# achraf-15/HiDeNN-FEM

Hardware: AMD Instinct MI355X
Metric: element-evals/sec (fwd+bwd energy) + achieved HBM GB/s, 2D quad mesh (higher is better)
Workload: dtype f64; 1 GPU; Example 4 (T1M x 1): 2D plate linear elasticity, 1000000 TRI3 (structured quads split in 2), 501501 nodes, gauss_order=4, r-adaptivity on, Neumann edges 500, fwd+bwd (loss + dX + dU); elements=1000000, nodes=501501, elements_per_gpu=1000000, tiles=1024, tile_elems=1200, element_order=paired slots, threads_per_tile=256, lds_bytes=38784, launch=hipgraph (1 x 1000 steps + 1 x 290), exchange=none, full=False

## Files before the change

hidenn_fem_amd/_lib.py:

```python
from __future__ import annotations

import ctypes as C
import os

import torch

_HERE = os.path.dirname(os.path.abspath(__file__))
LIB_PATH = os.path.join(_HERE, "csrc", "libhidenn_hip_lab.so" if os.environ.get("HFEM_LAB") == "1" else "libhidenn_hip.so")

_vp = C.c_void_p
_i32, _i64, _f64 = C.c_int32, C.c_int64, C.c_double


class PlanStats(C.Structure):
    _fields_ = [
        ("n_elems", _i64), ("n_nodes", _i64), ("n_edges", _i64),
        ("n_tiles", _i32), ("tile_elems", _i32),
        ("tile_elem_total", _i64), ("tile_node_total", _i64),
        ("max_tile_nodes", _i32), ("max_tile_owned", _i32),
        ("max_tile_elems", _i32), ("max_tile_edges", _i32),
        ("device_bytes", _i64), ("lds_bytes", _i32),
        ("shards", _i32), ("threads_per_tile", _i32), ("paired", _i32), ("slot_rows", _i32),
        ("store_policy", _i32), ("nodes_per_elem", _i32), ("row_line_factor", _f64),
    ]

    def as_dict(self):
        return {k: getattr(self, k) for k, _ in self._fields_}


class AdamTensor(C.Structure):
    _fields_ = [("p", _vp), ("g", _vp), ("m", _vp), ("v", _vp), ("n", _i64), ("lr", _f64), ("beta1", _f64),
                ("beta2", _f64), ("eps", _f64), ("dtype", _i32), ("block_begin", _i32)]


ADAM_TICKET_INTS = 1056


PROTOTYPES = {
    "hfem_version": (C.c_int, []),
    "hfem_last_error": (C.c_char_p, []),
    "hfem_device_count": (C.c_int, []),
    "hfem_tri3_energy_atomic": (C.c_int, [C.c_int, _vp, _vp, _vp, _i64, _i64, _i64, _vp, _f64, _vp, _vp, _vp, _vp, _vp]),
    "hfem_edge2_energy_atomic": (C.c_int, [C.c_int, _vp, _vp, _vp, _i64, _vp, _vp, _vp, _vp, _vp, _vp]),
    "hfem_plan_create": (C.c_int, [C.c_int, _vp, _i64, _i64, _vp, _vp, _vp, _vp, _i64, _i32, C.POINTER(_vp)]),
    "hfem_plan_create_ex": (C.c_int, [C.c_int, _vp, _i64, _i64, _i32, _vp, _vp, _vp, _vp, _i64, _i32, C.POINTER(_vp)]),
    "hfem_plan_destroy": (C.c_int, [_vp]),
    "hfem_plan_get_stats": (C.c_int, [_vp, C.POINTER(PlanStats)]),
    "hfem_plan_export": (_i64, [_vp, C.c_int, _vp, _i64]),
    "hfem_plan_serialize": (_i64, [_vp, _vp, _i64]),
    "hfem_plan_deserialize": (C.c_int, [C.c_int, _vp, _i64, C.POINTER(_vp)]),
    "hfem_tri3_energy_plan": (C.c_int, [_vp, _vp, _vp, _vp, _vp, _vp, _f64, _vp, _vp, _vp, _i32, _i32, _vp, _vp, _vp, _i32, _vp]),
    "hfem_tri3_energy_plan_f32": (C.c_int, [_vp, _vp, _vp, _vp, _vp, _vp, _f64, _vp, _vp, _vp, _i32, _i32, _vp, _vp, _vp, _i32, _vp]),
    "hfem_set_option": (C.c_int, [C.c_char_p, C.c_int]),
    "hfem_get_option": (C.c_int, [C.c_char_p]),
    "hfem_tri3_eval_fwd": (C.c_int, [C.c_int, _vp, _vp, _vp, _vp, _vp, _i64, _vp, _vp, _vp, _vp]),
    "hfem_tri3_eval_bwd": (C.c_int, [C.c_int, _vp, _vp, _vp, _vp, _vp, _i64, _vp, _vp, _vp, _vp, _vp, _vp]),
    "hfem_tri3_eval_fwd_conv": (C.c_int, [C.c_int, _vp, _vp, _vp, _vp, _vp, _i64, _vp, _vp, _vp, _i32, _vp]),
    "hfem_tri3_eval_bwd_conv": (C.c_int, [C.c_int, _vp, _vp, _vp, _vp, _vp, _i64, _vp, _vp, _vp, _vp, _vp, _i32, _vp]),
    "hfem_edge2_eval_fwd": (C.c_int, [C.c_int, _vp, _vp, _vp, _vp, _vp, _i64, _vp, _vp, _vp]),
    "hfem_edge2_eval_bwd": (C.c_int, [C.c_int, _vp, _vp, _vp, _vp, _vp, _i64, _vp, _vp, _vp, _vp, _vp]),
    "hfem_quad4_energy_atomic": (C.c_int, [C.c_int, _vp, _vp, _vp, _i64, _i64, _i64, _vp, _vp, _vp, _vp, _vp]),
    "hfem_adam_step_dev": (C.c_int, [C.c_int, _vp, _vp, _vp, _vp, _i64, _i32, C.c_double, C.c_double, C.c_double,
                                     C.c_double, _vp, _vp]),
    "hfem_counter_add": (C.c_int, [C.c_int, _vp, _i64, _vp]),
    "hfem_adam_multi_dev": (C.c_int, [C.c_int, _vp, _i32, _i32, _i64, _vp, _i64, _vp, _vp]),
    "hfem_lbfgs_create": (C.c_int, [C.c_int, _i64, _i32, _i32, C.POINTER(_vp)]),
    "hfem_lbfgs_destroy": (C.c_int, [_vp]),
    "hfem_lbfgs_check": (C.c_int, [_vp, _vp, _vp, _i32, C.c_double, C.c_double, _vp, _vp]),
    "hfem_lbfgs_direction": (C.c_int, [_vp, _vp, C.c_double, C.c_double, _vp]),
    "hfem_lbfgs_apply": (C.c_int, [_vp, _vp, _i64, _i64, _vp]),
    "hfem_lbfgs_direction_ptr": (_vp, [_vp]),
    "hfem_lbfgs_shard_payload_doubles": (_i64, [_vp]),
    "hfem_lbfgs_shard_gather": (C.c_int, [_vp, _vp, _vp, _i64, _vp, _vp, _i64, _vp, _vp]),
    "hfem_lbfgs_shard_local": (C.c_int, [_vp, _vp, _vp, _vp, _vp]),
    "hfem_lbfgs_shard_finish": (C.c_int, [_vp, _vp, _vp, _i32, _i32, _i32, _f64, _f64, _f64, _vp, _vp]),
    "hfem_lbfgs_shard_apply": (C.c_int, [_vp, _vp, _vp, _i64, _vp, _vp, _i64, _vp]),
    "hfem_lbfgs_shard_status": (C.c_int, [_vp, _vp, _vp]),
    "hfem_tri3_von_mises": (C.c_int, [C.c_int, _vp, _vp, _vp, _i64, C.c_double, C.c_double, _vp, _vp, _vp]),
    "hfem_line2_slopes": (C.c_int, [C.c_int, _vp, _vp, _i64, _i32, _vp, _vp]),
    "hfem_quad4_von_mises": (C.c_int, [C.c_int, _vp, _vp, _vp, _i64, C.c_double, C.c_double, _vp, _vp, _vp]),
    "hfem_tri3_stress_recover": (C.c_int, [C.c_int, _vp, _vp, _vp, _i64, _i64, _vp, _vp, _vp, _i32, _vp, _vp, _vp]),
    "hfem_quad4_stress_recover": (C.c_int, [C.c_int, _vp, _vp, _vp, _i64, _i64, _vp, _vp, _vp, _i32, _vp, _vp, _vp]),
    "hfem_tri3_zz_error": (C.c_int, [C.c_int, _vp, _vp, _vp, _i64, _vp, _vp, _i32, _vp, _vp, _vp, _vp, _vp]),
    "hfem_quad4_zz_error": (C.c_int, [C.c_int, _vp, _vp, _vp, _i64, _vp, _vp, _i32, _vp, _vp, _vp, _vp, _vp]),
    "hfem_tri3_hyper_energy_plan": (C.c_int, [_vp, _i32, _vp, _vp, _vp, _vp, _vp, _f64, _vp, _vp, _vp, _vp, _vp, _vp, _vp, _vp,
                                              _i32, _vp]),
    "hfem_quad4_hyper_energy_plan": (C.c_int, [_vp, _i32, _vp, _vp, _vp, _vp, _vp, _vp, _vp, _vp, _vp, _vp, _vp, _vp, _vp, _i32,
                                               _vp]),
    "hfem_tri3_energy_adam_step": (C.c_int, [_vp, _vp, _vp, _vp, _vp, _vp, _f64, _vp, _vp, _vp, _vp, _vp, _vp, _vp, _vp,
                                             _f64, _f64, _f64, _f64, _f64, _vp, _vp, _i32, _vp]),
    "hfem_tri3_energy_adam_step_ex": (C.c_int, [_vp, _i32, _vp, _vp, _vp, _vp, _vp, _f64, _vp, _vp, _vp, _vp, _vp, _vp, _vp, _vp,
                                                _vp, _f64, _f64, _f64, _f64, _f64, _vp, _i32, _i32, _vp, _i32, _vp]),
    "hfem_adam_prep": (C.c_int, [C.c_int, _vp, _f64, _f64, _vp, _vp]),
    "hfem_plan_loss_sum": (C.c_int, [_vp, _i32, _i32, _vp, _vp]),
    "hfem_iface_pack": (C.c_int, [C.c_int, _vp, _vp, _vp, _i32, _i32, _vp, _vp]),
    "hfem_iface_unpack": (C.c_int, [C.c_int, _vp, _vp, _vp, _i32, _i32, _vp, _vp, _i32, _i64, _i64, _vp, _vp]),
    "hfem_mg_load": (C.c_int, [C.c_char_p]),
    "hfem_mg_unique_id": (C.c_int, [_vp]),
    "hfem_mg_comm_create": (C.c_int, [C.c_int, C.c_int, C.c_int, _vp, C.POINTER(_vp)]),
    "hfem_mg_comm_destroy": (C.c_int, [_vp]),
    "hfem_mg_allreduce_sum": (C.c_int, [_vp, _vp, _vp, _i64, _vp]),
    "hfem_mg_allgather": (C.c_int, [_vp, _vp, _vp, _i64, _vp]),
    "hfem_adam_step_rows_dev": (C.c_int, [C.c_int, _vp, _vp, _vp, _vp, _vp, _i64, _f64, _f64, _f64, _f64, _vp, _vp]),
    "hfem_plan_set_span_stamps": (C.c_int, [_vp, _vp, _i64]),
    "hfem_peer_create": (C.c_int, [C.c_int, _i32, _i32, _i64, C.POINTER(_vp)]),
    "hfem_peer_ipc_handle": (C.c_int, [_vp, _vp]),
# ... 150 lines not shown
```

hidenn_fem_amd/csrc/build.py:

```python
from __future__ import annotations

import os
import subprocess
import sys
from concurrent.futures import ThreadPoolExecutor

HERE = os.path.dirname(os.path.abspath(__file__))
ROOT = os.path.dirname(os.path.dirname(HERE))
SOURCES = ["plan.cpp", "mg.cpp", "tri3_energy.hip", "tri3_stream.hip", "tri3_pair.hip", "tri3_pair_f32.hip", "tri3_pair_lab.hip", "tri3_pair_pipe.hip", "tri3_det.hip", "tri3_eval.hip", "line_rect.hip", "quad4.hip", "optim.hip", "exchange.hip", "peer.hip", "post.hip", "recover.hip", "lbfgs.hip", "cg.hip", "tri3_cg.hip", "quad4_cg.hip", "mesh_guard.hip", "amg.cpp", "tri3_amg.hip", "tri3_hyper.hip", "tri3_hyper_cg.hip", "quad4_hyper.hip", "quad4_hyper_cg.hip", "modal.hip"]
HEADERS = ["hfem_common.h", "hfem_amg.h", "hfem_amg_hyper_dev.h", "hfem_cg_dev.h", "hfem_crossing_dev.h", "hfem_device.h", "hfem_hyper_dev.h", "hfem_mesh_dev.h", "hfem_mesh_elem_dev.h", "hfem_plan_dev.h", "hfem_quad4_dev.h", "hfem_quad4_hyper_dev.h", "hfem_recover_hyper_dev.h", "tri3_energy_lab.inc", os.path.join(ROOT, "include", "hidenn_fem.h")]
OUT = os.path.join(HERE, "libhidenn_hip.so")
OUT_LAB = os.path.join(HERE, "libhidenn_hip_lab.so")
ARCH = "gfx950"
CXXFLAGS = ["-O3", "-std=c++17", "-fPIC", f"--offload-arch={ARCH}", "-munsafe-fp-atomics",
            "-ffp-contract=on", "-Wall", "-Wno-unused-function"]


def _stale(target, deps):
    if not os.path.exists(target):
        return True
    t = os.path.getmtime(target)
    return any(os.path.getmtime(d) > t for d in deps)


def build(force: bool = False, keep_temps: bool = False, lab: bool = False, tag: str = "", defines=()) -> str:
    hipcc = os.environ.get("HIPCC", "/opt/rocm/bin/hipcc")
    bdir = os.path.join(HERE, "build", "lab") if lab else os.path.join(HERE, "build")
    out = OUT_LAB if lab else OUT
    flags = CXXFLAGS + (["-DHFEM_LAB"] if lab else [])
    if tag:
        bdir, out = os.path.join(HERE, "build", tag), os.path.join(HERE, f"libhidenn_hip_{tag}.so")
        flags = flags + ["-D" + d for d in defines]
    srcs = [os.path.join(HERE, s) for s in SOURCES]
    hdrs = [h if os.path.isabs(h) else os.path.join(HERE, h) for h in HEADERS]
    objs = [os.path.join(bdir, os.path.splitext(s)[0] + ".o") for s in SOURCES]
    os.makedirs(bdir, exist_ok=True)

    def compile_one(pair):
        src, obj = pair
        res = obj + ".resource.txt"
        if not force and not _stale(obj, [src] + hdrs + [__file__]) and os.path.exists(res):
            return
        cmd = [hipcc] + flags + ["-x", "hip", "-c", src, "-o", obj, "-Rpass-analysis=kernel-resource-usage"]
        if keep_temps:
            cmd += ["-save-temps=obj"]
        r = subprocess.run(cmd, capture_output=True, text=True, cwd=bdir)
        if r.returncode != 0:
            raise RuntimeError(f"hipcc failed for {src}:\n{r.stdout}\n{r.stderr}")
        with open(res, "w") as f:
            f.write(r.stderr)

    with ThreadPoolExecutor(max_workers=4) as ex:
        list(ex.map(compile_one, zip(srcs, objs)))
    if force or _stale(out, objs):
        cmd = [hipcc, "-shared", "-fPIC", f"--offload-arch={ARCH}", "-o", out] + objs
        r = subprocess.run(cmd, capture_output=True, text=True)
        if r.returncode != 0:
            raise RuntimeError(f"link failed:\n{r.stdout}\n{r.stderr}")
    return out


def resource_usage(lab: bool = False):
    import re
    bdir = os.path.join(HERE, "build", "lab") if lab else os.path.join(HERE, "build")
    out = {}
    for s in SOURCES:
        path = os.path.join(bdir, os.path.splitext(s)[0] + ".o.resource.txt")
        if not os.path.exists(path):
            raise RuntimeError(f"{path} missing: run build() first")
        text = open(path).read()
        for blk in text.split("Function Name: ")[1:]:
            name = blk.split()[0]
            get = lambda key: int(re.search(key + r": (\d+)", blk).group(1))
            out[name] = dict(vgprs=get(r" VGPRs"), scratch=get(r"ScratchSize \[bytes/lane\]"), occupancy=get(r"Occupancy \[waves/SIMD\]"),
                             source=s)
    return out


if __name__ == "__main__":
    tag = sys.argv[sys.argv.index("--tag") + 1] if "--tag" in sys.argv else ""
    defs = [sys.argv[i + 1] for i, v in enumerate(sys.argv) if v == "--define"]
    print(build(force="--force" in sys.argv, keep_temps="--keep-temps" in sys.argv, lab="--lab" in sys.argv, tag=tag, defines=defs))
```

hidenn_fem_amd/csrc/hfem_common.h:

```cpp
#pragma once
#include <cstdint>
#include <cstdio>
#include <string>
#include <vector>

#include "../../include/hidenn_fem.h"

namespace hfem {

void set_error(const std::string &msg);
const char *get_error();

#define HFEM_ARG_CHECK(cond, msg)                                            \
    do {                                                                     \
        if (!(cond)) {                                                       \
            ::hfem::set_error(std::string(__func__) + ": " + (msg));         \
            return -1;                                                       \
        }                                                                    \
    } while (0)

constexpr int kLocalBits = 10;
constexpr int kMaxLocal = 1 << kLocalBits;
constexpr uint32_t kLocalMask = kMaxLocal - 1;
constexpr uint32_t kHomeBit = 1u << 30;
constexpr uint32_t kSkipBit = 1u << 31;
constexpr uint32_t kHasBBit = 1u << 10;
constexpr uint32_t kHomeBBit = 1u << 11;
constexpr uint32_t kChainedBit = 1u << 12;
constexpr int32_t kNodeTailPad = 2048;
constexpr int32_t kElemTailPad = 4096;
constexpr int32_t kMaxQuadSlots = 1024;

struct TileDesc {
    int32_t elem_off, n_elem;
    int32_t node_off, n_node;
    int32_t n_owned;
    int32_t edge_off, n_edge;
    int32_t pad;
};
static_assert(sizeof(TileDesc) == 32, "TileDesc must be 8 x int32");

struct HostPlan {
    int64_t ne = 0, nn = 0, ned = 0;
    int32_t tile_elems = 0;
    int32_t npe = 3;
    std::vector<TileDesc> tiles;
    std::vector<uint32_t> elem_pack;
    std::vector<uint32_t> elem_pack_hi;
    std::vector<int32_t> elem_gid;
    std::vector<int32_t> node_src;
    int32_t node_stride = 0, elem_stride = 0;
    int64_t elem_records = 0;
    int32_t col_stride = 0;
    int64_t node_records = 0;
    std::vector<uint32_t> edge_pack;
    std::vector<int32_t> edge_gid;
    int32_t max_nodes = 0, max_owned = 0, max_elems = 0, max_edges = 0;
    std::vector<int32_t> tile_chunks;
    std::vector<int32_t> elem_gid_b;
    bool paired = false;
    int64_t n_pairs = 0, n_chained = 0;
    int32_t max_rows = 0;
    std::vector<int32_t> conn32, x_src_g, u_src_g, edges32;
    int32_t max_chunk_elems = 0;
    int32_t shards = 1;
    std::vector<int32_t> shard_desc;
    int32_t pair_block = 256;
    std::vector<int32_t> owned_gid;
    std::vector<int32_t> owned_gid_by_slot;
};
constexpr int kChunks = 3;

int build_host_plan(const int64_t *conn, int npe, int64_t ne, int64_t nn, const double *coords,
                    const int32_t *x_src, const int32_t *u_src, const int64_t *edges,
                    int64_t ned, int32_t tile_elems, int32_t node_cap, int elem_order, int32_t chunk_cap,
                    HostPlan &out, int32_t pair_block = 256, int32_t shards = 1);

void serialize_host_plan(const HostPlan &h, const void *trailer, size_t trailer_bytes, std::vector<unsigned char> &blob);
int deserialize_host_plan(const void *blob, size_t n, HostPlan &h, void *trailer, size_t trailer_bytes);

void set_plan_curve(int c);
void set_plan_read_pack(int v);
void set_plan_snap(int percent);

}
```

hidenn_fem_amd/csrc/hfem_plan_dev.h:

```cpp
#pragma once
#include <hip/hip_runtime.h>

#include <mutex>
#include <vector>

#include "hfem_device.h"

namespace hfem {

struct PlanDev {
    const TileDesc *tiles;
    const uint32_t *elem_pack;
    const int2 *node_src;
    const uint32_t *edge_pack;
    const int32_t *edge_gid;
    const uint32_t *elem_pack_hi;
    const int4 *tile_chunks;
    int node_stride;
    int elem_stride;
    unsigned long long *span;
};

constexpr int kMaxPeers = 16;
constexpr size_t kPeerFlags = 0, kPeerData = 256;
// ... 201 lines not shown
    const int q = nb >> 3, r = nb & 7, x = b & 7;
    return x * q + min(x, r) + (b >> 3);
}

}

namespace hfem {
constexpr int kPipeMaxTiles = 16;
}

struct hfem_plan {
    hfem::HostPlan host;
    int device = -1;
    hfem::TileDesc *d_tiles = nullptr;
    uint32_t *d_elem_pack = nullptr;
    uint32_t *d_elem_pack_hi = nullptr;
    int2 *d_node_src = nullptr;
    uint32_t *d_edge_pack = nullptr;
    int32_t *d_edge_gid = nullptr;
    int4 *d_tile_chunks = nullptr;
    struct Det {
        int32_t *conn = nullptr, *x_src = nullptr, *u_src = nullptr, *edges = nullptr;
        int32_t *adj_ptr = nullptr, *adj = nullptr, *eadj_ptr = nullptr, *eadj = nullptr;
        double *partials = nullptr;
        int n_blocks = 0;
        bool ready = false;
    } det;
    double *d_partials = nullptr;
    std::mutex mu;
    int bank = 0;
    int prev_begin = 0, prev_n = 0;
    void *prev_stream = nullptr;
    struct Tune { int tiled_block = 512, store_policy = 16, tiled_fast = 1, fast_const_caps = 1, pair_tiles_per_wg = 1, pair_pipe_wps = 4; } tune;
    unsigned long long *d_stamps = nullptr;
    unsigned long long *span_buf = nullptr;
    int64_t span_slots = 0, span_next = 0;
    int64_t device_bytes = 0;
    double row_line_factor = 1.0;
    const hfem::PeerGetDev *peer_get = nullptr;
    const hfem::PeerPutDev *peer_put = nullptr;
    double *put_bc[2] = {nullptr, nullptr};
    const int32_t *put_pos[2] = {nullptr, nullptr};
    int peer_wait_begin = 0, peer_wait_end = 0;
    int32_t lds_bytes = 0;
    int32_t lds_bytes_pipe = 0;
};

namespace hfem {
inline PlanDev plan_dev(const hfem_plan *p) {
    return PlanDev{p->d_tiles, p->d_elem_pack, p->d_node_src, p->d_edge_pack, p->d_edge_gid, p->d_elem_pack_hi, p->d_tile_chunks, p->host.node_stride, p->host.elem_stride, nullptr};
}
inline Tri3Consts make_consts(const double mat[4], double W, const double Bk[6]) {
    Tri3Consts k;
    k.c11 = mat[0]; k.c12 = mat[1]; k.c22 = mat[2]; k.c33 = mat[3];
    k.W = W;
    for (int i = 0; i < 6; ++i) k.Bk[i] = Bk ? Bk[i] : 0.0;
    return k;
}
int launch_tri3_stream(const hfem_plan *plan, int n_grid, int tile_begin, const double *x_free, const double *x_fixed,
                       const double *u_free, const double *u_fixed, const Tri3Consts &kc, const double *T_edge,
                       double4 tc, double *partials, double *gx_free, double *gu_free, int skip_edges, int store_policy,
                       const LagSum &lag, hipStream_t s, int ablate = 0);
struct TileLaunch {
    PlanDev pd;
    int grid = 0, tile_begin = 0;
    const void *x_free = nullptr, *x_fixed = nullptr, *u_free = nullptr, *u_fixed = nullptr;
    Tri3Consts k;
    const double4 *T_edge = nullptr;
    double4 tc;
    double *partials = nullptr;
    void *gx = nullptr, *gu = nullptr;
    int max_nodes = 0, max_owned = 0, skip_edges = 0;
    int chain = -1;
    int lab_bits = 0;
    int col_stride = 256;
    unsigned long long *span = nullptr;
    unsigned long long *stamps = nullptr;
    size_t lds = 0;
    hipStream_t s = nullptr;
    int stagger = 0, stagger_cfg = 0x108;
};
int launch_tri3_pair(const hfem_plan *plan, TileLaunch A, int mode, bool hasb, bool phys, const LagSum &lag,
                     const AdamFuse &af);
int launch_tri3_pair_f32(const hfem_plan *plan, TileLaunch A, bool hasb, const LagSum &lag, const AdamFuse *adam = nullptr);
#ifdef HFEM_LAB
int launch_tri3_pair_lab(const hfem_plan *plan, TileLaunch A, int mode, bool hasb, bool phys, const LagSum &lag,
                         const AdamFuse &af);
#endif
int launch_tri3_pair_pipe(const hfem_plan *plan, TileLaunch A, int n_tiles, int tpw, const LagSum &lag);
int launch_tri3_det(hfem_plan *plan, const double *x_free, const double *x_fixed, const double *u_free,
                    const double *u_fixed, const Tri3Consts &kc, const double *T_edge, double4 tc, double *loss_out,
                    double *gx_free, double *gu_free, int skip_edges, bool phys, hipStream_t s);
void free_tri3_det(hfem_plan *plan);
int det_prepare(hfem_plan *plan, hipStream_t s);
int launch_iface_pack_sum(int dtype, const void *x_free, const void *u_free, const int32_t *rows, int n_x, int n_u, double *out,
                          int64_t loss_slot, const double *partials, int n_partials, int64_t *counter, double beta1,
                          double beta2, double *bc_next, hipStream_t s);
int launch_iface_put(const hfem_peer *peer, int dtype, const void *x_free, const void *u_free, const int32_t *rows, int n_x,
                     int n_u, int64_t loss_slot, const double *partials, int n_partials, int64_t *counter, double beta1,
                     double beta2, double *bc_next, hipStream_t s);
}
struct hfem_peer {
    int device = -1;
    int64_t stride = 0;
    size_t bytes = 0;
    char *local = nullptr;
    char *ctl = nullptr;
    hfem::PeerGetDev *get_dev = nullptr;
    hfem::PeerPutDev *put_dev = nullptr;
    const int32_t *put_pos[2] = {nullptr, nullptr};
    std::vector<void *> opened;
    bool connected = false;
    hfem::PeerView view{};
};
namespace hfem {
extern int g_quad4_stagger, g_quad4_stagger_shift, g_quad4_stagger_groups;
extern int g_quad4_ablate, g_quad4_pipe, g_quad4_const_caps, g_quad4_bits;

}
```

hidenn_fem_amd/csrc/plan.cpp:

```cpp
#include <algorithm>
#include <array>
#include <atomic>
#include <unordered_map>
#include <cstring>
#include <limits>
#include <numeric>

#include "hfem_common.h"

namespace hfem {

static thread_local std::string g_err;
void set_error(const std::string &msg) { g_err = msg; }
const char *get_error() { return g_err.c_str(); }

namespace {

inline uint32_t spread16(uint32_t v) {
    v &= 0xFFFFu;
    v = (v | (v << 8)) & 0x00FF00FFu;
    v = (v | (v << 4)) & 0x0F0F0F0Fu;
    v = (v | (v << 2)) & 0x33333333u;
    v = (v | (v << 1)) & 0x55555555u;
    return v;
// ... 344 lines not shown
            }
        telems.swap(out);
        return;
    }
    std::vector<std::vector<int32_t>> batch(nb);
    std::vector<std::vector<uint64_t>> used(nb, std::vector<uint64_t>(kMaxLocal / 64, 0));
    std::vector<int32_t> leftover;
    int start = 0;
    for (int i = 0; i < n; ++i) {
        const int32_t e = telems[i];
        int32_t l[3];
        for (int k = 0; k < 3; ++k) l[k] = lid[conn[3 * (int64_t)e + k]];
        int placed = -1;
        for (int t = 0; t < nb; ++t) {
            const int b = (start + t) % nb;
            const int cap = (b == nb - 1) ? n - 64 * (nb - 1) : 64;
            if ((int)batch[b].size() >= cap) continue;
            bool clash = false;
            for (int k = 0; k < 3; ++k)
                if (l[k] < n_owned && (used[b][l[k] >> 6] >> (l[k] & 63)) & 1) clash = true;
            if (clash) continue;
            placed = b;
            break;
        }
        if (placed < 0) { leftover.push_back(e); continue; }
        batch[placed].push_back(e);
        for (int k = 0; k < 3; ++k)
            if (l[k] < n_owned) used[placed][l[k] >> 6] |= 1ull << (l[k] & 63);
        start = (placed + 1) % nb;
    }
    size_t lo = 0;
    for (int b = 0; b < nb; ++b) {
        const int cap = (b == nb - 1) ? n - 64 * (nb - 1) : 64;
        while ((int)batch[b].size() < cap && lo < leftover.size()) batch[b].push_back(leftover[lo++]);
        out.insert(out.end(), batch[b].begin(), batch[b].end());
    }
    telems.swap(out);
}

void cut_tiles(const int64_t *conn, int npe, int64_t ne, int64_t nn, const std::vector<int32_t> &order, int32_t T,
               int32_t node_cap, std::vector<int64_t> &bounds) {
    bounds.assign(1, 0);
    if (node_cap <= 0) {
        for (int64_t p = T; p < ne; p += T) bounds.push_back(p);
        bounds.push_back(ne);
        return;
    }
    std::vector<int32_t> stamp(nn, -1);
    int32_t tile = 0, distinct = 0;
    int64_t start = 0;
    for (int64_t p = 0; p < ne; ++p) {
        const int64_t e = order[p];
        int fresh = 0;
        for (int k = 0; k < npe; ++k)
            if (stamp[conn[npe * e + k]] != tile) ++fresh;
        if (p > start && (p - start >= T || distinct + fresh > node_cap)) {
            int64_t cut = p;
            if (g_snap > 0 && (int64_t)g_codes.size() == ne) {
                const int64_t lo = std::max(start + 1, p - ((p - start) * g_snap) / 100);
                int best_lvl = -1;
                for (int64_t q = p; q >= lo; --q) {
                    const uint32_t x = g_codes[q - 1] ^ g_codes[q];
                    const int lvl = x ? (31 - __builtin_clz(x)) / 2 : -1;
                    if (lvl > best_lvl) { best_lvl = lvl; cut = q; }
                }
            }
            bounds.push_back(cut);
            ++tile;
            start = cut;
            distinct = 0;
            if (cut != p) { p = cut - 1; continue; }
        }
        for (int k = 0; k < npe; ++k) {
            int32_t &st = stamp[conn[npe * e + k]];
            if (st != tile) { st = tile; ++distinct; }
        }
    }
    bounds.push_back(ne);
}

int try_build(const int64_t *conn, int npe, int64_t ne, int64_t nn, const double *xy, const int32_t *x_src,
              const int32_t *u_src, const int64_t *edges, int64_t ned, int32_t T, int32_t node_cap,
              const std::vector<int32_t> &order, int elem_order, int32_t chunk_cap, int32_t pair_block, int32_t shards,
              HostPlan &P) {
    std::vector<int64_t> bounds;
    cut_tiles(conn, npe, ne, nn, order, T, node_cap, bounds);
    const int32_t nt_main = ne > 0 ? (int32_t)bounds.size() - 1 : 0;
    std::vector<int32_t> tile_of(ne);
    for (int32_t t = 0; t < nt_main; ++t)
        for (int64_t p = bounds[t]; p < bounds[t + 1]; ++p) tile_of[p] = t;
    std::vector<int32_t> owner(nn, std::numeric_limits<int32_t>::max());
    for (int64_t p = 0; p < ne; ++p) {
        const int32_t t = tile_of[p];
        const int64_t e = order[p];
        for (int k = 0; k < npe; ++k) {
            int32_t &o = owner[conn[npe * e + k]];
            if (t < o) o = t;
        }
    }
    int64_t n_orphan = 0;
    for (int64_t n = 0; n < nn; ++n)
        if (owner[n] == std::numeric_limits<int32_t>::max())
            owner[n] = nt_main + (int32_t)(n_orphan++ / kOrphanTileNodes);
    const int32_t nt = nt_main + (int32_t)((n_orphan + kOrphanTileNodes - 1) / kOrphanTileNodes);

    if (shards < 1) shards = 1;
    std::vector<int32_t> shard_of(nt, 0);
    std::vector<char> bnd(nt, 0);
    for (int32_t r = 0; r < shards; ++r)
        for (int64_t t = ((int64_t)nt * r) / shards; t < ((int64_t)nt * (r + 1)) / shards; ++t) shard_of[t] = r;

    std::vector<int64_t> adj_ptr(nn + 1, 0);
    for (int64_t e = 0; e < ne; ++e)
        for (int k = 0; k < npe; ++k) adj_ptr[conn[npe * e + k] + 1]++;
    for (int64_t n = 0; n < nn; ++n) adj_ptr[n + 1] += adj_ptr[n];
    std::vector<int32_t> adj(adj_ptr[nn]);
    {
        std::vector<int64_t> fill(adj_ptr.begin(), adj_ptr.end() - 1);
        for (int64_t p = 0; p < ne; ++p) {
            const int32_t e = order[p];
            for (int k = 0; k < npe; ++k) adj[fill[conn[npe * e + k]]++] = e;
        }
    }
    std::vector<int32_t> home(ne);
    for (int64_t p = 0; p < ne; ++p) home[order[p]] = tile_of[p];

    std::vector<int64_t> own_ptr(nt + 1, 0), edg_ptr(nt + 1, 0);
    for (int64_t n = 0; n < nn; ++n) own_ptr[owner[n] + 1]++;
    for (int64_t g = 0; g < ned; ++g) {
        const int32_t ti = owner[edges[2 * g]], tj = owner[edges[2 * g + 1]];
        edg_ptr[ti + 1]++;
        if (tj != ti) edg_ptr[tj + 1]++;
    }
    for (int32_t t = 0; t < nt; ++t) { own_ptr[t + 1] += own_ptr[t]; edg_ptr[t + 1] += edg_ptr[t]; }
    std::vector<int32_t> own(nn), tedge(edg_ptr[nt]);
    {
        std::vector<int64_t> f(own_ptr.begin(), own_ptr.end() - 1);
        for (int64_t n = 0; n < nn; ++n) own[f[owner[n]]++] = (int32_t)n;
        std::vector<int64_t> fe(edg_ptr.begin(), edg_ptr.end() - 1);
        for (int64_t g = 0; g < ned; ++g) {
            const int32_t ti = owner[edges[2 * g]], tj = owner[edges[2 * g + 1]];
            tedge[fe[ti]++] = (int32_t)g;
            if (tj != ti) tedge[fe[tj]++] = (int32_t)g;
        }
    }

    P = HostPlan();
    P.ne = ne; P.nn = nn; P.ned = ned; P.tile_elems = T; P.npe = npe;
    P.tiles.resize(nt);
    P.elem_pack.reserve(ne + ne / 4);
    P.elem_gid.reserve(ne + ne / 4);
    P.node_src.reserve(2 * (nn + nn / 3));

    bool by_row = false;
    if (x_src) {
        int32_t last = -1;
        for (int64_t n = 0; n < nn && !by_row; ++n)
            if (x_src[n] >= 0) { by_row = x_src[n] < last; last = x_src[n]; }
    }
    auto row_key = [&](int32_t n) -> int64_t { return x_src[n] >= 0 ? (int64_t)x_src[n] : ((int64_t)1 << 32) + (int64_t)(~x_src[n]); };
    auto by_row_less = [&](int32_t a, int32_t b) { return row_key(a) < row_key(b); };
    std::vector<int32_t> stamp_e(ne, -1), stamp_n(nn, -1), lid(nn, 0);
    std::vector<int32_t> first_use_stamp(elem_order == 4 ? nn : 0, -1), first_use(elem_order == 4 ? nn : 0, 0);
    std::vector<int32_t> telems, halo, own_order_buf;
    for (int32_t t = 0; t < nt; ++t) {
        TileDesc &d = P.tiles[t];
        d = TileDesc();
// ... 54 lines not shown
                    }
                    const bool along_x = (hi[0] - lo[0]) >= (hi[1] - lo[1]);
                    for (int i = 0; i < n; ++i) key[i] = {along_x ? cx[i] : cy[i], i};
                } else {
                    for (int i = 0; i < n; ++i) key[i] = {(double)i, i};
                }
                std::stable_sort(key.begin(), key.end());
                for (int r = 0; r < n; ++r) strip_of[key[r].second] = (int32_t)(((int64_t)r * kChunks) / std::max(n, 1));
            }
            for (int i = 0; i < n; ++i)
                for (int k = 0; k < npe; ++k) {
                    const int32_t nd = (int32_t)conn[npe * (int64_t)telems[i] + k];
                    if (first_use_stamp[nd] != t) { first_use_stamp[nd] = t; first_use[nd] = strip_of[i]; }
                    else first_use[nd] = std::min(first_use[nd], strip_of[i]);
                }
            auto fu = [&](int32_t nd) { return first_use_stamp[nd] == t ? first_use[nd] : kChunks - 1; };
            auto by_use = [&](int32_t a, int32_t b) { const int32_t fa = fu(a), fb = fu(b); return fa != fb ? fa < fb : a < b; };
            std::sort(own_order.begin(), own_order.end(), by_use);
            std::sort(halo.begin(), halo.end(), by_use);
            nloc = 0;
            for (int32_t nd : own_order) lid[nd] = nloc++;
            int32_t cnt_o[kChunks] = {0}, cnt_h[kChunks] = {0};
            for (int32_t nd : own_order) cnt_o[fu(nd)]++;
            for (int32_t nd : halo) cnt_h[fu(nd)]++;
            for (int32_t nd : halo) lid[nd] = nloc++;
            std::vector<int32_t> packed, part;
            int32_t ends[kChunks];
            for (int c = 0; c < kChunks; ++c) {
                part.clear();
                for (int i = 0; i < n; ++i)
                    if (strip_of[i] == c) part.push_back(telems[i]);
                pack_bank_groups(part, conn, npe, lid, d.n_owned, true, true, packed);
                ends[c] = (int32_t)packed.size();
                const int32_t len = ends[c] - (c ? ends[c - 1] : 0);
                if (chunk_cap > 0 && len > chunk_cap) return 1;
                P.max_chunk_elems = std::max(P.max_chunk_elems, len);
            }
            telems.swap(packed);
            const int32_t po0 = (cnt_o[0] + 63) / 64, po1 = (cnt_o[0] + cnt_o[1] + 63) / 64;
            const int32_t ph0 = (cnt_h[0] + 63) / 64, ph1 = (cnt_h[0] + cnt_h[1] + 63) / 64;
            chunk_rec[0] = ends[0]; chunk_rec[1] = ends[1];
            chunk_rec[2] = po0 | (po1 << 8) | (ph0 << 16) | (ph1 << 24);
        } else {
            for (int32_t n : halo) lid[n] = nloc++;
            if (!(elem_order >= 5 && npe == 3)) order_tile_elements(telems, conn, npe, lid, d.n_owned, elem_order);
        }
        nloc = d.n_owned + (int32_t)halo.size();
        if (elem_order == 4) P.tile_chunks.insert(P.tile_chunks.end(), chunk_rec, chunk_rec + 4);

        d.elem_off = (int32_t)P.elem_pack.size();
        d.node_off = (int32_t)(P.node_src.size() / 2);
        d.n_node = nloc;
        d.edge_off = (int32_t)P.edge_pack.size();
        d.n_edge = (int32_t)(edg_ptr[t + 1] - edg_ptr[t]);
        if (elem_order >= 5 && npe == 3) {
            const int n = (int)telems.size();
            std::unordered_map<uint64_t, int32_t> by_edge0;
            by_edge0.reserve((size_t)n * 2);
            for (int i = 0; i < n; ++i) {
                const int64_t e = telems[i];
                by_edge0[((uint64_t)conn[3 * e] << 32) | (uint32_t)conn[3 * e + 1]] = i;
            }
            std::vector<int32_t> succ(n, -1), pred(n, -1);
            for (int i = 0; i < n; ++i) {
                const int64_t e = telems[i];
                auto it = by_edge0.find(((uint64_t)conn[3 * e] << 32) | (uint32_t)conn[3 * e + 2]);
                if (it != by_edge0.end() && it->second != i && pred[it->second] < 0) { succ[i] = it->second; pred[it->second] = i; }
            }
            std::vector<char> used(n, 0);
            std::vector<std::array<int32_t, 2>> slots;
            slots.reserve(n);
            for (int pass = 0; pass < 2; ++pass)
                for (int i = 0; i < n; ++i) {
                    if (used[i] || (pass == 0 && pred[i] >= 0)) continue;
                    int a = i;
                    while (a >= 0 && !used[a]) {
                        used[a] = 1;
                        const int b = succ[a];
                        if (b >= 0 && !used[b]) { used[b] = 1; slots.push_back({a, b}); a = succ[b]; }
                        else { slots.push_back({a, -1}); a = -1; }
                    }
                }
            std::stable_sort(slots.begin(), slots.end(), [](const std::array<int32_t, 2> &x, const std::array<int32_t, 2> &y) { return (x[1] >= 0) > (y[1] >= 0); });
            std::vector<std::array<int32_t, 4>> items(slots.size());
            for (size_t s_ = 0; s_ < slots.size(); ++s_) {
                const int64_t ea = telems[slots[s_][0]];
                items[s_] = {lid[conn[3 * ea]], lid[conn[3 * ea + 1]], lid[conn[3 * ea + 2]],
                             slots[s_][1] >= 0 ? lid[conn[3 * (int64_t)telems[slots[s_][1]] + 2]] : -1};
            }
            std::vector<int32_t> order_s;
            std::vector<char> chain(slots.size(), 0);
            size_t n_pair = 0;
            while (n_pair < slots.size() && slots[n_pair][1] >= 0) ++n_pair;
            d.pad = pair_block;
            if (elem_order == 6 && pair_block != 256) { set_error("plan: the strip order (lab) needs 256-thread tiles"); return -1; }
            if (elem_order == 6) {
                const int S = (int)slots.size();
                const int H = std::min(kMaxRows, std::max(1, (S + 255) / 256));
                if (S > 256 * kMaxRows) return 1;
                auto gnode = [&](int si, int k) -> int64_t {
                    return k < 3 ? conn[3 * (int64_t)telems[slots[si][0]] + k] : conn[3 * (int64_t)telems[slots[si][1]] + 2];
                };
                std::unordered_map<uint64_t, int32_t> by_nd;
                by_nd.reserve(n_pair * 2);
                for (size_t si = 0; si < n_pair; ++si) by_nd[((uint64_t)gnode((int)si, 0) << 32) | (uint32_t)gnode((int)si, 3)] = (int32_t)si;
                std::vector<int32_t> nxt(n_pair, -1), prv(n_pair, -1);
                for (size_t si = 0; si < n_pair; ++si) {
                    auto it = by_nd.find(((uint64_t)gnode((int)si, 1) << 32) | (uint32_t)gnode((int)si, 2));
                    if (it != by_nd.end() && it->second != (int32_t)si && prv[it->second] < 0) { nxt[si] = it->second; prv[it->second] = (int32_t)si; }
                }
                std::vector<std::vector<int32_t>> strips, columns;
                {
                    const int L = H;
                    strips.clear();
                    std::vector<char> seen(n_pair, 0);
                    for (int pass = 0; pass < 2; ++pass)
                        for (size_t si = 0; si < n_pair; ++si) {
                            if (seen[si] || (pass == 0 && prv[si] >= 0)) continue;
                            int32_t a = (int32_t)si;
                            while (a >= 0 && !seen[a]) {
                                strips.emplace_back();
                                while (a >= 0 && !seen[a] && (int)strips.back().size() < L) { seen[a] = 1; strips.back().push_back(a); a = nxt[a]; }
                            }
                        }
                    std::stable_sort(strips.begin(), strips.end(), [](const std::vector<int32_t> &x, const std::vector<int32_t> &y) { return x.size() > y.size(); });
                    for (size_t si = n_pair; si < slots.size(); ++si) strips.push_back({(int32_t)si});
                    const int ncol = (S + H - 1) / H;
                    columns.assign(ncol, {});
                    std::vector<std::vector<int32_t>> with_room(H + 1);
                    for (int ci = ncol - 1; ci >= 0; --ci) with_room[H].push_back(ci);
                    for (size_t k = 0; k < strips.size(); ++k) {
                        std::vector<int32_t> st = strips[k];
                        while (!st.empty()) {
                            const int len = (int)st.size();
                            int r = len;
                            while (r <= H && with_room[r].empty()) ++r;
                            int take = len;
                            if (r > H) {
                                r = len - 1;
                                while (r > 0 && with_room[r].empty()) --r;
                                take = r;
                            }
                            if (r <= 0) return -1;
                            const int32_t ci = with_room[r].back();
                            with_room[r].pop_back();
                            columns[ci].insert(columns[ci].end(), st.begin(), st.begin() + take);
                            for (int q = 0; q + 1 < take; ++q) chain[st[q]] = 1;
                            if (r - take > 0) with_room[r - take].push_back(ci);
                            st.erase(st.begin(), st.begin() + take);
                        }
                    }
                    while (!columns.empty() && columns.back().empty()) columns.pop_back();
                }
                if (columns.size() > 256) return 1;
                auto shape = [&](const std::vector<int32_t> &c) { uint32_t v = 0; for (int32_t si : c) v = v * 4 + (chain[si] ? 3u : (slots[si][1] >= 0 ? 2u : 1u)); for (size_t q = c.size(); q < (size_t)kMaxRows; ++q) v *= 4; return v; };
                std::stable_sort(columns.begin(), columns.end(), [&](const std::vector<int32_t> &x, const std::vector<int32_t> &y) {
                    const uint32_t sx = shape(x), sy = shape(y);
                    return sx != sy ? sx > sy : gnode(x[0], 0) < gnode(y[0], 0);
                });
                std::vector<std::array<int32_t, 4 * kMaxRows>> citems(columns.size());
                int rows_used = 0;
                for (size_t ci = 0; ci < columns.size(); ++ci) {
                    citems[ci].fill(-1);
                    rows_used = std::max(rows_used, (int)columns[ci].size());
                    for (size_t r = 0; r < columns[ci].size(); ++r) {
                        const int32_t si = columns[ci][r];
                        citems[ci][4 * r + 0] = items[si][0];
                        citems[ci][4 * r + 3] = items[si][3];
                        if (!chain[si]) { citems[ci][4 * r + 1] = items[si][1]; citems[ci][4 * r + 2] = items[si][2]; }
                    }
                }
                std::vector<int32_t> corder;
                pack_column_groups(citems, d.n_owned, corder);
                const int stride = (int)((corder.size() + 15) / 16 * 16);
                d.pad = stride;
                order_s.assign((size_t)rows_used * stride, -1);
                for (size_t t_ = 0; t_ < corder.size(); ++t_)
                    for (size_t r = 0; r < columns[corder[t_]].size(); ++r) order_s[r * stride + t_] = columns[corder[t_]][r];
                while (!order_s.empty() && order_s.back() < 0) order_s.pop_back();
                P.max_rows = std::max(P.max_rows, rows_used);
            } else {
            if (g_halfwave_pack) {
                pack_slot_halfwaves(items, d.n_owned, order_s);
            } else {
                std::vector<std::array<int32_t, 4>> part(items.begin(), items.begin() + n_pair);
                std::vector<int32_t> o;
                pack_slot_groups(part, d.n_owned, o);
                while (!o.empty() && (o.size() & 15)) o.push_back(-1);
                order_s = o;
                part.assign(items.begin() + n_pair, items.end());
                o.clear();
                pack_slot_groups(part, d.n_owned, o);
                for (int32_t v : o) order_s.push_back(v < 0 ? -1 : v + (int32_t)n_pair);
            }
            P.max_rows = std::max(P.max_rows, ((int)order_s.size() + pair_block - 1) / pair_block);
            }
            d.n_elem = (int32_t)order_s.size();
            for (int32_t si : order_s) {
                if (si < 0) {
                    P.elem_pack.push_back(kSkipBit);
                    P.elem_pack_hi.push_back(0u);
                    P.elem_gid.push_back(-1);
                    P.elem_gid_b.push_back(-1);
                    continue;
                }
                const int32_t ea = telems[slots[si][0]], eb = slots[si][1] >= 0 ? telems[slots[si][1]] : -1;
                const std::array<int32_t, 4> &L = items[si];
                P.elem_pack.push_back((uint32_t)L[0] | ((uint32_t)L[1] << kLocalBits) | ((uint32_t)L[2] << (2 * kLocalBits)) |
                                      (home[ea] == t ? kHomeBit : 0u));
                P.elem_pack_hi.push_back(eb >= 0 ? ((uint32_t)L[3] | kHasBBit | (home[eb] == t ? kHomeBBit : 0u) | (chain[si] ? kChainedBit : 0u)) : 0u);
                P.elem_gid.push_back(ea);
                P.elem_gid_b.push_back(eb);
                P.n_pairs += eb >= 0;
                P.n_chained += chain[si];
            }
            P.paired = true;
        } else {
        d.n_elem = (int32_t)telems.size();
        for (int32_t e : telems) {
            if (e < 0) {
                P.elem_pack.push_back(kSkipBit);
                if (npe == 4) P.elem_pack_hi.push_back(0u);
                P.elem_gid.push_back(-1);
                continue;
            }
            const uint32_t l0 = lid[conn[npe * (int64_t)e]], l1 = lid[conn[npe * (int64_t)e + 1]],
                           l2 = lid[conn[npe * (int64_t)e + 2]];
            P.elem_pack.push_back(l0 | (l1 << kLocalBits) | (l2 << (2 * kLocalBits)) |
                                  (home[e] == t ? kHomeBit : 0u));
            if (npe == 4) P.elem_pack_hi.push_back((uint32_t)lid[conn[npe * (int64_t)e + 3]]);
            P.elem_gid.push_back(e);
        }
        }
        auto push_node = [&](int32_t n) {
            P.node_src.push_back(x_src ? x_src[n] : n);
            P.node_src.push_back(u_src ? u_src[n] : n);
        };
        for (int32_t n : own_order) { push_node(n); P.owned_gid_by_slot.push_back(n); }
        for (int32_t n : halo) { push_node(n); P.owned_gid_by_slot.push_back(n); }
        for (int64_t i = edg_ptr[t]; i < edg_ptr[t + 1]; ++i) {
            const int32_t g = tedge[i];
            const int64_t ni = edges[2 * (int64_t)g], nj = edges[2 * (int64_t)g + 1];
            P.edge_pack.push_back((uint32_t)lid[ni] | ((uint32_t)lid[nj] << kLocalBits) |
                                  (owner[ni] == t ? kHomeBit : 0u));
            P.edge_gid.push_back(g);
        }
        P.max_nodes = std::max(P.max_nodes, d.n_node);
        P.max_owned = std::max(P.max_owned, d.n_owned);
        P.max_elems = std::max(P.max_elems, d.n_elem);
        P.max_edges = std::max(P.max_edges, d.n_edge);
    }
    P.shards = shards;
    P.pair_block = pair_block;
    P.shard_desc.clear();
    {
        std::vector<TileDesc> sorted_tiles;
        std::vector<int32_t> sorted_chunks;
        const bool has_chunks = P.tile_chunks.size() == (size_t)4 * nt;
        sorted_tiles.reserve(nt);
        auto take = [&](int32_t t) {
            sorted_tiles.push_back(P.tiles[t]);
            if (has_chunks) sorted_chunks.insert(sorted_chunks.end(), P.tile_chunks.begin() + 4 * (size_t)t, P.tile_chunks.begin() + 4 * (size_t)t + 4);
        };
        for (int32_t r = 0; r < shards; ++r) {
            const int32_t lo = (int32_t)(((int64_t)nt * r) / shards), hi = (int32_t)(((int64_t)nt * (r + 1)) / shards);
            for (int32_t t = lo; t < hi; ++t)
                if (bnd[t]) take(t);
            const int32_t mid = (int32_t)sorted_tiles.size();
            for (int32_t t = lo; t < hi; ++t)
                if (!bnd[t]) take(t);
            P.shard_desc.insert(P.shard_desc.end(), {lo, mid, hi, 0});
        }
        if (shards > 1) {
            P.tiles.swap(sorted_tiles);
            if (has_chunks) P.tile_chunks.swap(sorted_chunks);
        }
    }
    {
        std::vector<int32_t> og;
        og.reserve(nn);
        for (const TileDesc &d : P.tiles)
            for (int32_t l = 0; l < d.n_owned; ++l) og.push_back(P.owned_gid_by_slot[(size_t)d.node_off + l]);
        P.owned_gid.swap(og);
    }
    {
        const int32_t stride = std::max(16, (P.max_nodes + 15) / 16 * 16);
        if ((int64_t)nt * stride + kNodeTailPad > (int64_t)std::numeric_limits<int32_t>::max()) {
            set_error("plan: tile arrays exceed int32 offsets");
            return -1;
        }
        std::vector<int32_t> ns((size_t)2 * ((size_t)nt * stride + kNodeTailPad));
        int32_t lastx = 0, lastu = 0;
        for (int32_t t = 0; t < nt; ++t) {
            TileDesc &d = P.tiles[t];
            const int32_t *srcp = P.node_src.data() + 2 * (size_t)d.node_off;
            int32_t *dst = ns.data() + 2 * (size_t)t * stride;
            std::memcpy(dst, srcp, sizeof(int32_t) * 2 * (size_t)d.n_node);
            if (d.n_node > 0) { lastx = srcp[2 * (d.n_node - 1)]; lastu = srcp[2 * (d.n_node - 1) + 1]; }
            else if (t == 0 && nt > 1 && P.tiles[1].n_node > 0) { lastx = P.node_src[2 * (size_t)P.tiles[1].node_off]; lastu = P.node_src[2 * (size_t)P.tiles[1].node_off + 1]; }
            for (int32_t l = d.n_node; l < stride; ++l) { dst[2 * l] = lastx; dst[2 * l + 1] = lastu; }
            d.node_off = t * stride;
        }
        for (size_t l = (size_t)nt * stride; l < (size_t)nt * stride + kNodeTailPad; ++l) { ns[2 * l] = lastx; ns[2 * l + 1] = lastu; }
        P.node_records = (int64_t)P.node_src.size() / 2;
        P.node_src.swap(ns);
        P.node_stride = stride;
    }
    {
        int32_t cs = 0;
        if (P.paired) {
            for (int32_t t = 0; t < nt; ++t) cs = std::max(cs, P.tiles[t].pad);
            P.max_elems = 0;
            for (int32_t t = 0; t < nt; ++t) {
                const TileDesc &d = P.tiles[t];
                const int32_t ne_new = d.n_elem > 0 ? ((d.n_elem - 1) / d.pad) * cs + (d.n_elem - 1) % d.pad + 1 : 0;
                P.max_elems = std::max(P.max_elems, ne_new);
            }
            P.col_stride = cs;
        }
        const int64_t stride = std::max(16, (P.max_elems + 15) / 16 * 16);
        const size_t total = (size_t)nt * stride + kElemTailPad;
        if (total > (size_t)std::numeric_limits<int32_t>::max()) { set_error("plan: tile arrays exceed int32 offsets"); return -1; }
        const bool hi = !P.elem_pack_hi.empty(), gb = !P.elem_gid_b.empty();
        std::vector<uint32_t> ep(total, kSkipBit), eh(hi ? total : 0, 0u);
        std::vector<int32_t> eg(total, -1), egb(gb ? total : 0, -1);
        int64_t real = 0;
        for (int32_t t = 0; t < nt; ++t) {
            TileDesc &d = P.tiles[t];
            const size_t so = (size_t)d.elem_off, dn = (size_t)t * stride, n = (size_t)d.n_elem;
            int32_t n_new = 0;
            for (size_t i = 0; i < n; ++i) {
                const size_t k = cs > 0 ? (i / d.pad) * cs + i % d.pad : i;
                ep[dn + k] = P.elem_pack[so + i];
                eg[dn + k] = P.elem_gid[so + i];
                if (hi) eh[dn + k] = P.elem_pack_hi[so + i];
                if (gb) egb[dn + k] = P.elem_gid_b[so + i];
                n_new = (int32_t)k + 1;
            }
            real += d.n_elem;
            d.elem_off = (int32_t)dn;
            d.n_elem = n_new;
            if (cs > 0) d.pad = cs;
        }
        P.elem_pack.swap(ep); P.elem_gid.swap(eg); P.elem_pack_hi.swap(eh); P.elem_gid_b.swap(egb);
        P.elem_stride = (int32_t)stride;
        P.elem_records = real;
    }
    if (P.elem_pack.size() > (size_t)std::numeric_limits<int32_t>::max() ||
        P.node_src.size() / 2 > (size_t)std::numeric_limits<int32_t>::max()) {
        set_error("plan: tile arrays exceed int32 offsets");
        return -1;
    }
    return 0;
}

}

void set_plan_curve(int c) { set_locality_curve(c); }
void set_plan_snap(int percent) { set_tile_snap(percent); }
void set_plan_read_pack(int v) { set_halfwave_pack(v); }

int build_host_plan(const int64_t *conn, int npe, int64_t ne, int64_t nn, const double *coords,
                    const int32_t *x_src, const int32_t *u_src, const int64_t *edges,
                    int64_t ned, int32_t tile_elems, int32_t node_cap, int elem_order, int32_t chunk_cap,
                    HostPlan &out, int32_t pair_block, int32_t shards) {
    if (pair_block != 256 && pair_block != 512) { set_error("plan: pair_block must be 256 or 512"); return -1; }
    if (shards < 1 || shards > 4096) { set_error("plan: shards must be in [1, 4096]"); return -1; }
    if (npe != 3 && npe != 4) { set_error("plan: nodes per element must be 3 (TRI3) or 4 (QUAD4)"); return -1; }
    if (ne < 0 || nn < 0 || ned < 0 || nn > std::numeric_limits<int32_t>::max() ||
        ne > std::numeric_limits<int32_t>::max() || ned > std::numeric_limits<int32_t>::max()) {
        set_error("plan: sizes must be in [0, 2^31)");
        return -1;
    }
    if ((ne > 0 && !conn) || (ned > 0 && !edges)) { set_error("plan: null connectivity/edges"); return -1; }
    for (int64_t i = 0; i < npe * ne; ++i)
        if (conn[i] < 0 || conn[i] >= nn) { set_error("plan: connectivity index out of range"); return -1; }
    for (int64_t i = 0; i < 2 * ned; ++i)
        if (edges[i] < 0 || edges[i] >= nn) { set_error("plan: edge index out of range"); return -1; }
    if (tile_elems <= 0) tile_elems = 1024;
    if (tile_elems > 4096) tile_elems = 4096;

    std::vector<int32_t> order;
    morton_order(conn, npe, ne, nn, coords, order);
    for (int32_t T = tile_elems; T >= 16; T = (T * 2) / 3) {
        const int rc = try_build(conn, npe, ne, nn, coords, x_src, u_src, edges, ned, T, node_cap, order, elem_order, chunk_cap,
                                 pair_block, shards, out);
        if (rc == 0 && npe == 4 && out.max_elems > kMaxQuadSlots) continue;
        if (rc == 0 && out.paired && out.max_rows > (pair_block == 512 ? 2 : kMaxRows)) continue;
        if (rc == 0) {
            out.conn32.assign(conn, conn + npe * ne);
            out.edges32.assign(edges, edges + 2 * ned);
            out.x_src_g.resize(nn);
            out.u_src_g.resize(nn);
            for (int64_t n = 0; n < nn; ++n) {
                out.x_src_g[n] = x_src ? x_src[n] : (int32_t)n;
                out.u_src_g[n] = u_src ? u_src[n] : (int32_t)n;
            }
        }
        if (rc <= 0) return rc;
    }
    set_error("plan: could not fit a tile into 1024 local nodes / element slots (node valence too high?)");
    return -1;
}

namespace {
constexpr uint32_t kBlobVersion = 1;
struct BlobScalars {
    int64_t ne, nn, ned, elem_records, node_records, n_pairs, n_chained;
    int32_t tile_elems, npe, node_stride, elem_stride, col_stride, max_nodes, max_owned, max_elems, max_edges, max_rows,
        max_chunk_elems, shards, pair_block, paired;
};
uint64_t fnv1a(const unsigned char *p, size_t n) {
    uint64_t h = 1469598103934665603ull;
    size_t i = 0;
    for (; i + 8 <= n; i += 8) {
        uint64_t w;
        std::memcpy(&w, p + i, 8);
        h = (h ^ w) * 1099511628211ull;
    }
    for (; i < n; ++i) h = (h ^ p[i]) * 1099511628211ull;
    return h;
}
template <typename T>
void put_vec(std::vector<unsigned char> &b, const std::vector<T> &v) {
    const uint64_t n = v.size();
    const size_t nb = (size_t)n * sizeof(T), at = b.size();
    b.resize(at + 8 + ((nb + 7) & ~(size_t)7), 0);
    std::memcpy(b.data() + at, &n, 8);
    if (nb) std::memcpy(b.data() + at + 8, v.data(), nb);
}
template <typename T>
bool get_vec(const unsigned char *p, size_t n, size_t &at, std::vector<T> &v) {
    if (at + 8 > n) return false;
    uint64_t cnt;
    std::memcpy(&cnt, p + at, 8);
    if (cnt > (n - at - 8) / sizeof(T)) return false;
    const size_t nb = (size_t)cnt * sizeof(T);
    v.resize((size_t)cnt);
    if (nb) std::memcpy(v.data(), p + at + 8, nb);
    at += 8 + ((nb + 7) & ~(size_t)7);
    return at <= n;
}
}

void serialize_host_plan(const HostPlan &h, const void *trailer, size_t trailer_bytes, std::vector<unsigned char> &b) {
    b.clear();
    b.insert(b.end(), {'H', 'F', 'E', 'M', 'P', 'L', 'A', 'N'});
    const uint32_t head[2] = {kBlobVersion, (uint32_t)trailer_bytes};
    b.insert(b.end(), (const unsigned char *)head, (const unsigned char *)head + 8);
    BlobScalars sc{};
    sc.ne = h.ne; sc.nn = h.nn; sc.ned = h.ned; sc.elem_records = h.elem_records; sc.node_records = h.node_records;
    sc.n_pairs = h.n_pairs; sc.n_chained = h.n_chained; sc.tile_elems = h.tile_elems; sc.npe = h.npe;
    sc.node_stride = h.node_stride; sc.elem_stride = h.elem_stride; sc.col_stride = h.col_stride; sc.max_nodes = h.max_nodes;
    sc.max_owned = h.max_owned; sc.max_elems = h.max_elems; sc.max_edges = h.max_edges; sc.max_rows = h.max_rows;
    sc.max_chunk_elems = h.max_chunk_elems; sc.shards = h.shards; sc.pair_block = h.pair_block; sc.paired = h.paired ? 1 : 0;
    b.insert(b.end(), (const unsigned char *)&sc, (const unsigned char *)&sc + sizeof(sc));
    b.resize((b.size() + 7) & ~(size_t)7, 0);
    std::vector<int32_t> td((const int32_t *)h.tiles.data(), (const int32_t *)h.tiles.data() + 8 * h.tiles.size());
    put_vec(b, td);
    put_vec(b, h.elem_pack); put_vec(b, h.elem_pack_hi); put_vec(b, h.elem_gid); put_vec(b, h.elem_gid_b);
    put_vec(b, h.node_src); put_vec(b, h.edge_pack); put_vec(b, h.edge_gid); put_vec(b, h.tile_chunks);
    put_vec(b, h.conn32); put_vec(b, h.x_src_g); put_vec(b, h.u_src_g); put_vec(b, h.edges32);
    put_vec(b, h.shard_desc); put_vec(b, h.owned_gid);
    const size_t at = b.size();
    b.resize(at + ((trailer_bytes + 7) & ~(size_t)7), 0);
    if (trailer_bytes) std::memcpy(b.data() + at, trailer, trailer_bytes);
    const uint64_t sum = fnv1a(b.data(), b.size());
    b.insert(b.end(), (const unsigned char *)&sum, (const unsigned char *)&sum + 8);
}

int deserialize_host_plan(const void *blob, size_t n, HostPlan &h, void *trailer, size_t trailer_bytes) {
    const unsigned char *p = (const unsigned char *)blob;
    if (!p || n < 24 + sizeof(BlobScalars) || std::memcmp(p, "HFEMPLAN", 8) != 0) { set_error("plan blob: not a plan blob"); return -1; }
    uint32_t head[2];
    std::memcpy(head, p + 8, 8);
    if (head[0] != kBlobVersion) { set_error("plan blob: written by another format version"); return -1; }
    if (head[1] != trailer_bytes) { set_error("plan blob: written by another library version (trailer size)"); return -1; }
    uint64_t sum;
    std::memcpy(&sum, p + n - 8, 8);
    if (sum != fnv1a(p, n - 8)) { set_error("plan blob: checksum mismatch (truncated or corrupted)"); return -1; }
    size_t at = 16;
    BlobScalars sc;
    std::memcpy(&sc, p + at, sizeof(sc));
    at = (at + sizeof(sc) + 7) & ~(size_t)7;
    h = HostPlan();
    h.ne = sc.ne; h.nn = sc.nn; h.ned = sc.ned; h.elem_records = sc.elem_records; h.node_records = sc.node_records;
    h.n_pairs = sc.n_pairs; h.n_chained = sc.n_chained; h.tile_elems = sc.tile_elems; h.npe = sc.npe;
    h.node_stride = sc.node_stride; h.elem_stride = sc.elem_stride; h.col_stride = sc.col_stride; h.max_nodes = sc.max_nodes;
    h.max_owned = sc.max_owned; h.max_elems = sc.max_elems; h.max_edges = sc.max_edges; h.max_rows = sc.max_rows;
    h.max_chunk_elems = sc.max_chunk_elems; h.shards = sc.shards; h.pair_block = sc.pair_block; h.paired = sc.paired != 0;
    std::vector<int32_t> td;
    bool ok = get_vec(p, n - 8, at, td) && td.size() % 8 == 0;
    ok = ok && get_vec(p, n - 8, at, h.elem_pack) && get_vec(p, n - 8, at, h.elem_pack_hi) && get_vec(p, n - 8, at, h.elem_gid) &&
         get_vec(p, n - 8, at, h.elem_gid_b) && get_vec(p, n - 8, at, h.node_src) && get_vec(p, n - 8, at, h.edge_pack) &&
         get_vec(p, n - 8, at, h.edge_gid) && get_vec(p, n - 8, at, h.tile_chunks) && get_vec(p, n - 8, at, h.conn32) &&
         get_vec(p, n - 8, at, h.x_src_g) && get_vec(p, n - 8, at, h.u_src_g) && get_vec(p, n - 8, at, h.edges32) &&
         get_vec(p, n - 8, at, h.shard_desc) && get_vec(p, n - 8, at, h.owned_gid);
    ok = ok && at + ((trailer_bytes + 7) & ~(size_t)7) == n - 8;
    if (!ok) { set_error("plan blob: malformed"); return -1; }
    h.tiles.resize(td.size() / 8);
    if (!td.empty()) std::memcpy((void *)h.tiles.data(), td.data(), td.size() * 4);
    if (trailer_bytes) std::memcpy(trailer, p + at, trailer_bytes);
    const size_t nt = h.tiles.size();
    if ((h.npe != 3 && h.npe != 4) || h.node_stride < 0 || h.elem_stride < 0 || h.max_nodes > kMaxLocal ||
        h.node_src.size() < 2 * (nt * (size_t)h.node_stride) || h.elem_pack.size() < nt * (size_t)h.elem_stride ||
        ((h.npe == 4 || h.paired) && h.elem_pack_hi.size() != h.elem_pack.size()) || (int64_t)h.conn32.size() != h.npe * h.ne ||
        (int64_t)h.x_src_g.size() != h.nn || (int64_t)h.u_src_g.size() != h.nn || (int64_t)h.edges32.size() != 2 * h.ned ||
        h.shard_desc.size() != 4 * (size_t)std::max(1, h.shards)) {
        set_error("plan blob: inconsistent array sizes");
        return -1;
    }
    for (const TileDesc &d : h.tiles)
        if (d.n_node < 0 || d.n_node > h.max_nodes || d.n_owned < 0 || d.n_owned > d.n_node || d.n_elem < 0 || d.n_elem > h.max_elems ||
            d.node_off < 0 || (size_t)d.node_off + d.n_node > h.node_src.size() / 2 || d.elem_off < 0 ||
            (size_t)d.elem_off + d.n_elem > h.elem_pack.size() || d.n_edge < 0 || d.edge_off < 0 ||
            (size_t)d.edge_off + d.n_edge > h.edge_pack.size()) {
            set_error("plan blob: tile descriptor out of range");
            return -1;
        }
    return 0;
}

}
```

hidenn_fem_amd/csrc/tri3_energy.hip:

```cpp
#include <hip/hip_runtime.h>

#include <algorithm>
#include <atomic>
#include <cstring>
#include <memory>
#include <mutex>
#include <type_traits>

#include "hfem_device.h"
#include "hfem_plan_dev.h"

#ifdef HFEM_LAB
#define HFEM_LAB_SECTION 0
#include "tri3_energy_lab.inc"
#undef HFEM_LAB_SECTION
#else
#define HFEM_LAB_TILED_STAGGER(stagger_ticks, stagger_mode)
#define HFEM_LAB_FAST_STAGGER(stagger_ticks, stagger_cfg)
#endif

namespace hfem {

constexpr int kBlock = 256;

// ... 298 lines not shown
#pragma unroll
        for (int j = 0; j < NPT; ++j) {
            const int l = tid + j * BLOCK;
            if (l < n_owned) {
                const int2 rows = src[l];
                if (rows.x >= 0) adam_fused_row<V2>(af, 0, rows.x, acc0[l], acc1[l], nd_xy[l], bc1, sqrt_bc2);
                if (rows.y >= 0) adam_fused_row<V2>(af, 1, rows.y, acc2[l], acc3[l], nd_uv[l], bc1, sqrt_bc2);
            }
        }
    } else {
    typedef unsigned int u32x4 __attribute__((ext_vector_type(4)));
    typedef unsigned int u32x2 __attribute__((ext_vector_type(2)));
    constexpr bool kWide = sizeof(V2) == 16;
    __amdgpu_buffer_rsrc_t rx, ru;
    if (SP != 0) {
        rx = __builtin_amdgcn_make_buffer_rsrc((void *)gx_free, 0, 0x7FFFFFF0, 0x00020000);
        ru = __builtin_amdgcn_make_buffer_rsrc((void *)gu_free, 0, 0x7FFFFFF0, 0x00020000);
    }
#pragma unroll
    for (int j = 0; j < NPT; ++j) {
        const int l = tid + j * BLOCK;
        if (l < n_owned) {
            if (gx_free && s[j].x >= 0) {
                V2 v;
                v.x = acc0[l]; v.y = acc1[l];
                if (SP == 0) gx_free[s[j].x] = v;
                else if (kWide) __builtin_amdgcn_raw_buffer_store_b128(*reinterpret_cast<const u32x4 *>(&v), rx, s[j].x * 16, 0, SP);
                else __builtin_amdgcn_raw_buffer_store_b64(*reinterpret_cast<const u32x2 *>(&v), rx, s[j].x * 8, 0, SP);
            }
            if (gu_free && s[j].y >= 0) {
                V2 v;
                v.x = acc2[l]; v.y = acc3[l];
                if (SP == 0) gu_free[s[j].y] = v;
                else if (kWide) __builtin_amdgcn_raw_buffer_store_b128(*reinterpret_cast<const u32x4 *>(&v), ru, s[j].y * 16, 0, SP);
                else __builtin_amdgcn_raw_buffer_store_b64(*reinterpret_cast<const u32x2 *>(&v), ru, s[j].y * 8, 0, SP);
            }
        }
    }
    }
    HFEM_FSTAMP(6)
    if (tid == 0) {
        double tile_e = 0.0;
#pragma unroll
        for (int w = 0; w < BLOCK / 64; ++w) tile_e += red[w];
        partials[slot] = tile_e;
    }
    HFEM_FSTAMP(7)
#undef HFEM_FSTAMP
}

#ifdef HFEM_LAB
#define HFEM_LAB_SECTION 1
#include "tri3_energy_lab.inc"
#undef HFEM_LAB_SECTION
#endif

__global__ __launch_bounds__(kBlock) void sum_partials_kernel(const double *__restrict__ partials, int n,
                                                             double *__restrict__ out) {
    __shared__ double red[kBlock / 64];
    double v = 0.0;
    for (int i = threadIdx.x; i < n; i += kBlock) v += partials[i];
    const double tot = block_sum(v, red);
    if (threadIdx.x == 0) out[0] = tot;
}

}
using namespace hfem;

namespace {
struct Defaults {
    std::atomic<int> tiled_block{512};
    std::atomic<int> store_policy{-1};
    std::atomic<int> tiled_fast{1};
    std::atomic<int> fast_const_caps{1};
    std::atomic<int> pair_pipe_wps{4};
    std::atomic<int> pair_tiles_per_wg{1};
    std::atomic<int> plan_elem_order{-1};
    std::atomic<int> plan_node_cap{-1};
    std::atomic<int> plan_read_pack{2};
    std::atomic<int> plan_snap{0};
    std::atomic<int> plan_chunk_cap{512};
    std::atomic<int> plan_shards{1};
    std::atomic<int> plan_pair_block{-1};
} g_def;

#ifdef HFEM_LAB
#define HFEM_LAB_SECTION 2
#include "tri3_energy_lab.inc"
#undef HFEM_LAB_SECTION
#endif

hfem_plan::Tune current_tune() {
    hfem_plan::Tune t;
    t.tiled_block = g_def.tiled_block.load();
    t.store_policy = g_def.store_policy.load();
    t.tiled_fast = g_def.tiled_fast.load();
    t.fast_const_caps = g_def.fast_const_caps.load();
    t.pair_tiles_per_wg = g_def.pair_tiles_per_wg.load();
    t.pair_pipe_wps = g_def.pair_pipe_wps.load();
    return t;
}

int grid_for(int64_t n, int cap = 256 * 8) {
    int64_t g = (n + kBlock - 1) / kBlock;
    if (g < 1) g = 1;
    if (g > cap) g = cap;
    return (int)g;
}

TileLaunch tile_launch(const hfem_plan *plan, const void *x_free, const void *x_fixed, const void *u_free, const void *u_fixed,
                       const double mat[4], double W, const double Bk[6], const double *T_edge, const double Tconst[4],
                       int tile_begin, void *gx, void *gu, int flags, hipStream_t s) {
    TileLaunch A;
    A.pd = plan_dev(plan); A.tile_begin = tile_begin;
    A.x_free = x_free; A.x_fixed = x_fixed; A.u_free = u_free; A.u_fixed = u_fixed;
    A.k = make_consts(mat, W, Bk); A.T_edge = (const double4 *)T_edge;
    A.tc = Tconst ? make_double4(Tconst[0], Tconst[1], Tconst[2], Tconst[3]) : make_double4(0, 0, 0, 0);
    A.gx = (flags & HFEM_FLAG_NO_GX) ? nullptr : gx; A.gu = (flags & HFEM_FLAG_NO_GU) ? nullptr : gu;
    A.max_nodes = plan->host.max_nodes; A.max_owned = plan->host.max_owned; A.skip_edges = (flags & HFEM_FLAG_NO_EDGES) ? 1 : 0;
    A.stamps = plan->d_stamps; A.lds = (size_t)plan->lds_bytes; A.s = s;
    return A;
}

bool has_body_force(const double Bk[6]) {
    for (int i = 0; Bk && i < 6; ++i)
        if (Bk[i] != 0.0) return true;
    return false;
}

template <int BLK, int NPT, int EPT, bool HB, int SP, typename V2, int CO, bool ADAM, bool PHYS, bool STAMP = false>
void launch_fast(const TileLaunch &A, int grid, const AdamFuse &af, const LagSum &lag) {
    const size_t lds = CO > 0 ? (size_t)(A.max_nodes * 32 + CO * 32 + 128) : A.lds;
    if constexpr (!HB && !PHYS && !STAMP && BLK == 512 && (SP == 16 || SP == 2)) {
        if (lag.pg_blocks) {
            hipLaunchKernelGGL((tri3_energy_fast_kernel<BLK, NPT, EPT, HB, STAMP, SP, V2, 0, CO, ADAM, PHYS, true>), dim3(grid), dim3(BLK),
                               lds, A.s, A.pd, A.tile_begin, (V2 *)const_cast<void *>(A.x_free), (const V2 *)A.x_fixed, (V2 *)const_cast<void *>(A.u_free),
                               (const V2 *)A.u_fixed, A.k, A.T_edge, A.tc, A.partials, (V2 *)A.gx, (V2 *)A.gu, A.max_nodes,
                               CO > 0 ? CO : A.max_owned, A.skip_edges, A.stagger, A.stagger_cfg, A.stamps, af, lag);
            return;
        }
    }
    hipLaunchKernelGGL((tri3_energy_fast_kernel<BLK, NPT, EPT, HB, STAMP, SP, V2, 0, CO, ADAM, PHYS>), dim3(grid), dim3(BLK),
                       lds, A.s, A.pd, A.tile_begin, (const V2 *)A.x_free, (const V2 *)A.x_fixed, (const V2 *)A.u_free,
                       (const V2 *)A.u_fixed, A.k, A.T_edge, A.tc, A.partials, (V2 *)A.gx, (V2 *)A.gu, A.max_nodes,
                       CO > 0 ? CO : A.max_owned, A.skip_edges, A.stagger, A.stagger_cfg, A.stamps, af, lag);
}

template <int BLK>
void launch_generic(const TileLaunch &A, int grid) {
    hipLaunchKernelGGL((tri3_energy_tiled_kernel<BLK, 0>), dim3(grid), dim3(BLK), A.lds, A.s, A.pd, A.tile_begin,
                       (const double2 *)A.x_free, (const double2 *)A.x_fixed, (const double2 *)A.u_free,
                       (const double2 *)A.u_fixed, A.k, A.T_edge, A.tc, A.partials, (double2 *)A.gx, (double2 *)A.gu,
                       A.max_nodes, A.max_owned, A.skip_edges, 0, 0, A.stamps);
}

bool launch_fast_f64(const hfem_plan *plan, const TileLaunch &A, int n, bool hasb, const LagSum &lag) {
    const HostPlan &h = plan->host;
    const int blk = plan->tune.tiled_block, sp = plan->tune.store_policy;
    const int n_lag = n + (lag.prev ? 1 : 0) + lag.pg_blocks;
    if (lag.pg_blocks && !(blk == 512 && !hasb && (sp == 16 || sp == 2))) return false;
    if (plan->tune.fast_const_caps && blk == 512 && !hasb && (sp == 16 || sp == 2) && h.max_nodes > 512 && h.max_owned <= 560 &&
        h.max_nodes * 32 + 560 * 32 + 128 <= 38912 && h.max_elems <= 3 * 512) {
        if (sp == 2) launch_fast<512, 2, 3, false, 2, double2, 560, false, false>(A, n_lag, AdamFuse{}, lag);
        else launch_fast<512, 2, 3, false, 16, double2, 560, false, false>(A, n_lag, AdamFuse{}, lag);
        return true;
    }
    if (sp == 2 && blk == 512 && !hasb && h.max_nodes <= 2 * 512 && h.max_elems <= 4 * 512) {
        if (h.max_elems <= 3 * 512) launch_fast<512, 2, 3, false, 2, double2, 0, false, false>(A, n_lag, AdamFuse{}, lag);
        else launch_fast<512, 2, 4, false, 2, double2, 0, false, false>(A, n_lag, AdamFuse{}, lag);
        return true;
    }
#define HFEM_FAST_HB(BLK, NPT, EPT)                                                                                       \
    {                                                                                                                     \
// ... 138 lines not shown
    if (plan->device >= 0) {
        (void)hipSetDevice(plan->device);
        (void)hipFree(plan->d_tiles);
        (void)hipFree(plan->d_elem_pack);
        (void)hipFree(plan->d_elem_pack_hi);
        (void)hipFree(plan->d_node_src);
        (void)hipFree(plan->d_edge_pack);
        (void)hipFree(plan->d_edge_gid);
        (void)hipFree(plan->d_tile_chunks);
        free_tri3_det(plan);
        (void)hipFree(plan->d_partials);
        (void)hipFree(plan->d_stamps);
    }
    delete plan;
    return 0;
}

namespace {
int finalize_plan(std::unique_ptr<hfem_plan> &p, int device) {
    const HostPlan &h = p->host;
    p->lds_bytes = h.max_nodes * 32 + h.max_owned * 32 + 128;
    p->lds_bytes_pipe = p->lds_bytes + 32 * kPipeMaxTiles + (h.npe == 4 ? 8 : 4) * ((h.max_elems + 3) & ~3);
    if (device >= 0) {
        if (int rc = use_device(device)) return rc;
        p->device = device;
        hfem_plan *raw = p.get();
        int rc = 0;
        if (!rc) rc = hfem_upload(&raw->d_tiles, h.tiles.data(), h.tiles.size(), raw->device_bytes);
        if (!rc) rc = hfem_upload(&raw->d_elem_pack, h.elem_pack.data(), h.elem_pack.size(), raw->device_bytes);
        if (!rc && (h.npe == 4 || h.paired)) rc = hfem_upload(&raw->d_elem_pack_hi, h.elem_pack_hi.data(), h.elem_pack_hi.size(), raw->device_bytes);
        if (!rc) rc = hfem_upload(&raw->d_node_src, h.node_src.data(), h.node_src.size() / 2, raw->device_bytes);
        if (!rc) rc = hfem_upload(&raw->d_edge_pack, h.edge_pack.data(), h.edge_pack.size(), raw->device_bytes);
        if (!rc) rc = hfem_upload(&raw->d_edge_gid, h.edge_gid.data(), h.edge_gid.size(), raw->device_bytes);
        if (!rc && !h.tile_chunks.empty()) rc = hfem_upload(&raw->d_tile_chunks, h.tile_chunks.data(), h.tile_chunks.size() / 4, raw->device_bytes);
        if (!rc) rc = hfem_upload(&raw->d_partials, nullptr, 2 * h.tiles.size(), raw->device_bytes);
        HFEM_LAB_UPLOAD_STAMPS(raw, h, rc)
        if (!rc && p->lds_bytes > 64 * 1024) {
            set_error("plan: tile needs more than 64 KiB of LDS");
            rc = -1;
        }
        if (rc) { hfem_plan_destroy(p.release()); return rc; }
    }
    return 0;
}
}

extern "C" int hfem_plan_create(int device, const int64_t *conn, int64_t ne, int64_t nn,
                                const double *coords_hint, const int32_t *x_src, const int32_t *u_src,
                                const int64_t *edges, int64_t ned, int32_t tile_elems, hfem_plan **out) {
    return hfem_plan_create_ex(device, conn, ne, nn, 3, coords_hint, x_src, u_src, edges, ned, tile_elems, out);
}

extern "C" int hfem_plan_create_ex(int device, const int64_t *conn, int64_t ne, int64_t nn, int32_t nodes_per_elem,
                                   const double *coords_hint, const int32_t *x_src, const int32_t *u_src,
                                   const int64_t *edges, int64_t ned, int32_t tile_elems, hfem_plan **out) {
    HFEM_ARG_CHECK(out, "null out pointer");
    *out = nullptr;
    std::unique_ptr<hfem_plan> p(new hfem_plan);
    p->tune = current_tune();
    const bool auto_store = p->tune.store_policy < 0;
    if (auto_store) p->tune.store_policy = nn >= 750000 ? 2 : 16;
    int32_t node_cap = g_def.plan_node_cap.load();
    const int32_t shards = std::max(1, g_def.plan_shards.load());
    int32_t pair_block = g_def.plan_pair_block.load();
    const int64_t per_shard = ne / shards;
    if (node_cap < 0) {
        node_cap = 0;
        if (tile_elems <= 0) {
            node_cap = 557;
            if (nodes_per_elem == 3 && per_shard <= 600000) {
                if (pair_block < 0) pair_block = per_shard > 100000 ? 512 : 256;
                if (per_shard <= 200000) node_cap = pair_block == 512 ? 430 : 208;
            }
        }
    }
    if (pair_block < 0) pair_block = 256;
    if (tile_elems <= 0) tile_elems = node_cap > 0 ? 1200 : 1024;
    int order = g_def.plan_elem_order.load();
#ifndef HFEM_LAB
    HFEM_ARG_CHECK(!(order == 6 && device >= 0), "plan_elem_order 6 (pairs chained into strips): device plans in the lab build only (libhidenn_hip_lab.so)");
#endif
    const bool auto_order = order < 0;
    if (auto_order) order = nodes_per_elem == 3 ? 5 : 3;
    if (build_host_plan(conn, nodes_per_elem, ne, nn, coords_hint, x_src, u_src, edges, ned, tile_elems, node_cap, order,
                        g_def.plan_chunk_cap.load(), p->host, pair_block, shards))
        return -1;
    if (auto_order && p->host.paired && 2 * p->host.n_pairs * 10 < 7 * ne) {
        p->host = HostPlan();
        if (build_host_plan(conn, nodes_per_elem, ne, nn, coords_hint, x_src, u_src, edges, ned, tile_elems, node_cap, 3,
                            g_def.plan_chunk_cap.load(), p->host, 256, shards))
            return -1;
    }
    const HostPlan &h = p->host;
    {
        double acc = 0.0;
        int64_t cnt = 0;
        std::vector<int32_t> lines;
        for (const TileDesc &d : h.tiles) {
            lines.clear();
            for (int32_t l = 0; l < d.n_node; ++l) {
                const int32_t r = h.node_src[2 * ((size_t)d.node_off + l)];
                if (r >= 0) lines.push_back(r >> 3);
            }
            if (lines.empty()) continue;
            const size_t rows = lines.size();
            std::sort(lines.begin(), lines.end());
            const size_t distinct = std::unique(lines.begin(), lines.end()) - lines.begin();
            acc += (double)distinct / (double)((rows + 7) / 8);
            ++cnt;
        }
        p->row_line_factor = cnt ? acc / (double)cnt : 1.0;
    }
    if (auto_store && p->tune.store_policy == 2 && p->row_line_factor > 2.5) p->tune.store_policy = 16;
    if (int rc = finalize_plan(p, device)) return rc;
    *out = p.release();
    return 0;
}

namespace {
struct PlanTrailer {
    int32_t tiled_block, store_policy, tiled_fast, fast_const_caps, pair_tiles_per_wg, pair_pipe_wps;
    int32_t hfem_version, reserved;
    double row_line_factor;
};
}

extern "C" int64_t hfem_plan_serialize(const hfem_plan *plan, void *buf, int64_t cap_bytes) {
    if (!plan) { set_error("hfem_plan_serialize: null plan"); return -1; }
    PlanTrailer t{plan->tune.tiled_block, plan->tune.store_policy, plan->tune.tiled_fast, plan->tune.fast_const_caps,
                  plan->tune.pair_tiles_per_wg, plan->tune.pair_pipe_wps, HFEM_VERSION, 0, plan->row_line_factor};
    std::vector<unsigned char> blob;
    serialize_host_plan(plan->host, &t, sizeof(t), blob);
    if (buf) {
        if (cap_bytes < (int64_t)blob.size()) { set_error("hfem_plan_serialize: buffer too small"); return -1; }
        std::memcpy(buf, blob.data(), blob.size());
    }
    return (int64_t)blob.size();
}

extern "C" int hfem_plan_deserialize(int device, const void *blob, int64_t n_bytes, hfem_plan **out) {
    HFEM_ARG_CHECK(out, "null out pointer");
    *out = nullptr;
    HFEM_ARG_CHECK(blob && n_bytes > 0, "empty blob");
    std::unique_ptr<hfem_plan> p(new hfem_plan);
    PlanTrailer t{};
    if (deserialize_host_plan(blob, (size_t)n_bytes, p->host, &t, sizeof(t))) return -1;
    HFEM_ARG_CHECK(t.hfem_version == HFEM_VERSION, "plan blob written by another library version: rebuild the plan");
    p->tune.tiled_block = t.tiled_block; p->tune.store_policy = t.store_policy; p->tune.tiled_fast = t.tiled_fast;
    p->tune.fast_const_caps = t.fast_const_caps; p->tune.pair_tiles_per_wg = t.pair_tiles_per_wg; p->tune.pair_pipe_wps = t.pair_pipe_wps;
    p->row_line_factor = t.row_line_factor;
    if (int rc = finalize_plan(p, device)) return rc;
    *out = p.release();
    return 0;
}

extern "C" int hfem_plan_get_stats(const hfem_plan *plan, hfem_plan_stats *out) {
    HFEM_ARG_CHECK(plan && out, "null pointer");
    const HostPlan &h = plan->host;
    std::memset(out, 0, sizeof(*out));
    out->n_elems = h.ne; out->n_nodes = h.nn; out->n_edges = h.ned;
    out->n_tiles = (int32_t)h.tiles.size();
    out->tile_elems = h.tile_elems;
    out->tile_elem_total = h.elem_records;
    out->tile_node_total = h.node_records;
    out->max_tile_nodes = h.max_nodes; out->max_tile_owned = h.max_owned;
    out->max_tile_elems = h.max_elems; out->max_tile_edges = h.max_edges;
    out->device_bytes = plan->device_bytes;
    out->lds_bytes = plan->lds_bytes;
    out->shards = h.shards;
    out->threads_per_tile = h.paired ? h.pair_block : (h.npe == 4 ? 256 : plan->tune.tiled_block);
    out->paired = h.paired ? 1 : 0;
    out->slot_rows = h.paired ? h.max_rows : 0;
    out->store_policy = plan->tune.store_policy;
    out->nodes_per_elem = h.npe;
    out->row_line_factor = plan->row_line_factor;
    return 0;
}

extern "C" int64_t hfem_plan_export(const hfem_plan *plan, int which, void *buf, int64_t cap_elems) {
    if (!plan) { set_error("hfem_plan_export: null plan"); return -1; }
    const HostPlan &h = plan->host;
    const void *src = nullptr;
    int64_t n = 0;
    size_t esz = 4;
    switch (which) {
        case 0: src = h.tiles.data(); n = (int64_t)h.tiles.size() * 8; break;
        case 1: src = h.elem_pack.data(); n = (int64_t)h.elem_pack.size(); break;
        case 2: src = h.node_src.data(); n = (int64_t)h.node_src.size(); break;
        case 3: src = h.edge_pack.data(); n = (int64_t)h.edge_pack.size(); break;
        case 4: src = h.edge_gid.data(); n = (int64_t)h.edge_gid.size(); break;
        case 5: src = h.elem_gid.data(); n = (int64_t)h.elem_gid.size(); break;
        case 7: src = h.elem_pack_hi.data(); n = (int64_t)h.elem_pack_hi.size(); break;
        case 8: src = h.tile_chunks.data(); n = (int64_t)h.tile_chunks.size(); break;
        case 9: src = h.elem_gid_b.data(); n = (int64_t)h.elem_gid_b.size(); break;
        case 10: src = h.shard_desc.data(); n = (int64_t)h.shard_desc.size(); break;
        case 11: src = h.owned_gid.data(); n = (int64_t)h.owned_gid.size(); break;
        case 6: {
            n = (int64_t)h.tiles.size() * 32;
            if (buf) {
                if (cap_elems < n || plan->device < 0 || !plan->d_stamps) { set_error("hfem_plan_export: stamps need the lab build, a device plan and a buffer"); return -1; }
                (void)hipSetDevice(plan->device);
                if (hipMemcpy(buf, plan->d_stamps, (size_t)n * 4, hipMemcpyDeviceToHost) != hipSuccess) { set_error("hfem_plan_export: stamp copy failed"); return -1; }
            }
            return n;
        }
        default: set_error("hfem_plan_export: unknown array id"); return -1;
    }
    if (buf) {
        if (cap_elems < n) { set_error("hfem_plan_export: buffer too small"); return -1; }
        if (n) std::memcpy(buf, src, (size_t)n * esz);
    }
    return n;
}

extern "C" int hfem_tri3_energy_plan(hfem_plan *plan, const double *x_free, const double *x_fixed,
                                     const double *u_free, const double *u_fixed, const double mat[4],
                                     double W, const double Bk[6], const double *T_edge,
                                     const double Tconst[4], int32_t tile_begin, int32_t tile_end,
                                     double *loss_out, double *gx_free, double *gu_free, int32_t flags,
                                     void *stream) {
    HFEM_ARG_CHECK(plan && mat && loss_out, "null pointer");
    HFEM_ARG_CHECK(plan->device >= 0, "host-only plan (created with device < 0) cannot launch");
    HFEM_ARG_CHECK(plan->host.npe == 3, "this plan was built for QUAD4: use hfem_quad4_energy_plan");
    HFEM_ARG_CHECK(x_free && u_free, "x_free / u_free must be given");
    const HostPlan &h = plan->host;
    if (int rc = tile_range(plan, __func__, tile_begin, tile_end)) return rc;
    HFEM_ARG_CHECK(h.ned == 0 || T_edge || Tconst, "plan has Neumann edges: need a traction table");
    if (int rc = use_device(plan->device)) return rc;
    PlanLock lock(plan);
    HFEM_LAB_REFRESH_TUNE(plan)
    const int nt = (int)h.tiles.size(), n = tile_end - tile_begin;
    TileLaunch A = tile_launch(plan, x_free, x_fixed, u_free, u_fixed, mat, W, Bk, T_edge, Tconst, tile_begin, gx_free, gu_free,
                               flags, (hipStream_t)stream);
    const bool hasb = has_body_force(Bk);
    const bool phys = (flags & HFEM_FLAG_PHYSICAL_GRAD) != 0;
    const bool phys_fast = phys && !(flags & HFEM_FLAG_DETERMINISTIC) &&
                           (h.paired || (plan->tune.tiled_block == 512 && h.max_nodes <= 2 * 512 && h.max_elems <= 4 * 512));
    if ((flags & HFEM_FLAG_DETERMINISTIC) || (phys && !phys_fast)) {
        HFEM_ARG_CHECK(tile_begin == 0 && tile_end == nt, "HFEM_FLAG_DETERMINISTIC / physical fallback: whole plan only");
        HFEM_ARG_CHECK(!(flags & (HFEM_FLAG_NO_LOSS_SUM | HFEM_FLAG_SUM_PREVIOUS | HFEM_FLAG_PEER_GET)), "HFEM_FLAG_DETERMINISTIC always delivers the loss and has no in-launch get");
        return launch_tri3_det(plan, x_free, x_fixed, u_free, u_fixed, A.k, T_edge, A.tc, loss_out, (double *)A.gx, (double *)A.gu,
                               A.skip_edges, phys, A.s);
    }
    const bool lag_consume = (flags & HFEM_FLAG_SUM_PREVIOUS) != 0;
    LossBanks banks;
    LagSum lag;
    if (int rc = banks.begin(plan, __func__, flags, tile_begin, n, stream, loss_out, lag)) return rc;
    HFEM_ARG_CHECK(!lag_consume || h.paired || (plan->tune.tiled_fast && plan->tune.tiled_block == 512 && !hasb && !phys && plan->tune.store_policy != 0 &&
                   h.max_nodes <= 1024 && h.max_elems <= 2048),
                   "HFEM_FLAG_SUM_PREVIOUS: only the default (register-prefetched, 512-thread) kernel path implements it");
    if (flags & HFEM_FLAG_PEER_GET)
        if (int rc = peer_get_fill(plan, __func__, !hasb && !phys, n, lag)) return rc;
    int n_partials = n;
    if (n > 0) {
        A.partials = banks.partials; A.grid = n + (lag.prev ? 1 : 0) + lag.pg_blocks;
        bool launched = false;
        HFEM_LAB_TRI3_LAUNCH(plan, A, n, hasb, phys, lag, n_partials, launched)
        if (!launched && h.paired) {
// ... 238 lines not shown
                                        (plan->tune.store_policy == 16 || plan->tune.store_policy == 2)),
                   "the in-launch get needs the paired-slot kernel's plain slot loop (no chained records) or the 512-thread "
                   "one-element-per-slot kernel with write-through / nt stores");
    plan->peer_get = peer->get_dev; plan->peer_wait_begin = wait_begin; plan->peer_wait_end = wait_end;
    return 0;
}

extern "C" int hfem_plan_set_peer_put(hfem_plan *plan, hfem_peer *peer, double *bc_a, double *bc_b) {
    HFEM_ARG_CHECK(plan, "null pointer");
    PlanLock lock(plan);
    if (!peer) { plan->peer_put = nullptr; plan->put_bc[0] = plan->put_bc[1] = nullptr; plan->put_pos[0] = plan->put_pos[1] = nullptr; return 0; }
    HFEM_ARG_CHECK(peer->connected && peer->put_dev, "hfem_peer_connect / hfem_peer_attach_put first");
    HFEM_ARG_CHECK(peer->device == plan->device, "plan and peer windows live on different devices");
    HFEM_ARG_CHECK(plan->host.paired && plan->host.n_chained == 0, "the in-launch put needs a paired-slot plan (plain slot loop)");
    HFEM_ARG_CHECK(bc_a && bc_b && bc_a != bc_b, "need two distinct bias-correction buffers");
    plan->peer_put = peer->put_dev; plan->put_bc[0] = bc_a; plan->put_bc[1] = bc_b;
    plan->put_pos[0] = peer->put_pos[0]; plan->put_pos[1] = peer->put_pos[1];
    return 0;
}

static int plan_iface_put_any(int dtype, hfem_plan *plan, hfem_peer *peer, int32_t tile_begin, int32_t tile_end,
                              const void *x_free, const void *u_free, const int32_t *rows, int32_t n_x, int32_t n_u,
                              int64_t loss_slot, int64_t *counter, double beta1, double beta2, double *bc_next, void *stream) {
    HFEM_ARG_CHECK(plan && peer, "null pointer");
    HFEM_ARG_CHECK(plan->device >= 0, "host-only plan (created with device < 0) cannot launch");
    HFEM_ARG_CHECK(peer->connected, "hfem_peer_connect has not been called");
    HFEM_ARG_CHECK(peer->device == plan->device, "plan and peer windows live on different devices");
    HFEM_ARG_CHECK(n_x >= 0 && n_u >= 0 && loss_slot >= n_x + n_u && loss_slot < peer->stride, "bad sizes");
    HFEM_ARG_CHECK((n_x + n_u == 0 || rows) && (n_x == 0 || x_free) && (n_u == 0 || u_free), "null pointer");
    if (int rc = tile_range(plan, __func__, tile_begin, tile_end)) return rc;
    if (int rc = use_device(plan->device)) return rc;
    PlanLock lock(plan);
    return launch_iface_put(peer, dtype, x_free, u_free, rows, n_x, n_u, loss_slot, bank_ptr(plan, plan->bank) + tile_begin,
                            tile_end - tile_begin, counter, beta1, beta2, bc_next, (hipStream_t)stream);
}

extern "C" int hfem_plan_iface_put(hfem_plan *plan, hfem_peer *peer, int32_t tile_begin, int32_t tile_end,
                                   const double *x_free, const double *u_free, const int32_t *rows, int32_t n_x, int32_t n_u,
                                   int64_t loss_slot, int64_t *counter, double beta1, double beta2, double *bc_next,
                                   void *stream) {
    return plan_iface_put_any(0, plan, peer, tile_begin, tile_end, x_free, u_free, rows, n_x, n_u, loss_slot, counter, beta1, beta2,
                              bc_next, stream);
}

extern "C" int hfem_plan_iface_put_f32(hfem_plan *plan, hfem_peer *peer, int32_t tile_begin, int32_t tile_end,
                                       const float *x_free, const float *u_free, const int32_t *rows, int32_t n_x, int32_t n_u,
                                       int64_t loss_slot, int64_t *counter, double beta1, double beta2, double *bc_next,
                                       void *stream) {
    return plan_iface_put_any(1, plan, peer, tile_begin, tile_end, x_free, u_free, rows, n_x, n_u, loss_slot, counter, beta1, beta2,
                              bc_next, stream);
}

extern "C" int hfem_set_option(const char *name, int value) {
    HFEM_ARG_CHECK(name, "null option name");
    const std::string n(name);
    if (n == "tiled_block") {
        HFEM_ARG_CHECK(value == 256 || value == 512 || value == 1024, "tiled_block must be 256, 512 or 1024");
        g_def.tiled_block = value;
    } else if (n == "store_policy") {
        HFEM_ARG_CHECK(value == -1 || value == 0 || value == 2 || value == 16 || value == 17 || value == 18,
                       "store_policy: -1 (by mesh size, default), 16 (sc1 write-through), 2 (nt), 0 (plain), 17 (sc0 sc1), 18 (sc1 nt)");
        g_def.store_policy = value;
    } else if (n == "tiled_fast") {
        g_def.tiled_fast = value ? 1 : 0;
    } else if (n == "fast_const_caps") {
        g_def.fast_const_caps = value ? 1 : 0;
    } else if (n == "quad4_const_caps") {
        g_quad4_const_caps = value ? 1 : 0;
    } else if (n == "plan_elem_order") {
        HFEM_ARG_CHECK(value >= -1 && value <= 6, "plan_elem_order must be -1 (auto) or 0..6");
        g_def.plan_elem_order = value;
    } else if (n == "plan_node_cap") {
        HFEM_ARG_CHECK(value >= -1 && value <= 1024, "plan_node_cap must be -1 (auto), 0 (off) or 1..1024");
        g_def.plan_node_cap = value;
    } else if (n == "plan_chunk_cap") {
        HFEM_ARG_CHECK(value >= 0 && value <= 4096, "plan_chunk_cap: 0 (no limit) .. 4096 slots");
        g_def.plan_chunk_cap = value;
    } else if (n == "plan_shards") {
        HFEM_ARG_CHECK(value >= 1 && value <= 4096, "plan_shards: 1 .. 4096 ranks");
        g_def.plan_shards = value;
    } else if (n == "plan_pair_block") {
        HFEM_ARG_CHECK(value == -1 || value == 256 || value == 512, "plan_pair_block: -1 (auto), 256 or 512 threads per tile");
        g_def.plan_pair_block = value;
    } else if (n == "plan_curve") {
        HFEM_ARG_CHECK(value == 0 || value == 1, "plan_curve: 0 Morton, 1 Hilbert");
        set_plan_curve(value);
    } else if (n == "plan_read_pack") {
        g_def.plan_read_pack = value;
        set_plan_read_pack(value);
    } else if (n == "plan_snap") {
        HFEM_ARG_CHECK(value >= 0 && value <= 50, "plan_snap: 0..50 (percent of a tile)");
        g_def.plan_snap = value;
        set_plan_snap(value);
#ifdef HFEM_LAB
#define HFEM_LAB_SECTION 4
#include "tri3_energy_lab.inc"
#undef HFEM_LAB_SECTION
#endif
    } else {
        set_error("hfem_set_option: unknown option '" + n + "' (lab knobs need libhidenn_hip_lab.so)");
        return -1;
    }
    return 0;
}

extern "C" int hfem_get_option(const char *name) {
    if (!name) return -1;
    const std::string n(name);
    if (n == "tiled_block") return g_def.tiled_block.load();
    if (n == "store_policy") return g_def.store_policy.load();
    if (n == "tiled_fast") return g_def.tiled_fast.load();
    if (n == "fast_const_caps") return g_def.fast_const_caps.load();
    if (n == "pair_tiles_per_wg") return g_def.pair_tiles_per_wg.load();
    if (n == "pair_pipe_wps") return g_def.pair_pipe_wps.load();
    if (n == "quad4_const_caps") return g_quad4_const_caps;
    if (n == "plan_elem_order") return g_def.plan_elem_order.load();
    if (n == "plan_node_cap") return g_def.plan_node_cap.load();
    if (n == "plan_chunk_cap") return g_def.plan_chunk_cap.load();
    if (n == "plan_shards") return g_def.plan_shards.load();
    if (n == "plan_pair_block") return g_def.plan_pair_block.load();
    if (n == "plan_snap") return g_def.plan_snap.load();
    if (n == "plan_read_pack") return g_def.plan_read_pack.load();
    if (n == "lab_build") {
#ifdef HFEM_LAB
        return 1;
#else
        return 0;
#endif
    }
#ifdef HFEM_LAB
#define HFEM_LAB_SECTION 5
#include "tri3_energy_lab.inc"
#undef HFEM_LAB_SECTION
#endif
    return -1;
}
```

hidenn_fem_amd/csrc/tri3_pair.hip:

```cpp
#include <hip/hip_runtime.h>

#include <type_traits>

#include "hfem_device.h"
#include "hfem_plan_dev.h"

namespace hfem {

template <int BLOCK, int NPT, int EPT, int WPS, int CAPO, bool HASB = false, bool PHYS = false, typename V2 = double2,
          bool ADAM = false, bool CHAIN = false, int CAPN = 0, int SP = 16, bool PG = false>
__global__ __launch_bounds__(BLOCK, WPS) void tri3_energy_pair_kernel(
    PlanDev pd, int tile_begin, typename RowArg<V2, PG>::type x_free, const V2 *__restrict__ x_fixed,
    typename RowArg<V2, PG>::type u_free, const V2 *__restrict__ u_fixed, Tri3Consts k,
    const double4 *__restrict__ T_edge, double4 Tconst, double *__restrict__ partials,
    V2 *__restrict__ gx_free, V2 *__restrict__ gu_free, int cap_nodes, int cap_owned_rt, int skip_edges,
    LagSum lag, AdamFuse af, int col_stride) {
    const int cap_owned = CAPO > 0 ? CAPO : cap_owned_rt;
    const int cap_n = CAPN > 0 ? CAPN : cap_nodes;
    extern __shared__ double2 lds[];
    double2 *nd_xy = lds;
    double2 *nd_uv = lds + cap_n;
    double *acc0 = reinterpret_cast<double *>(lds + 2 * cap_n);
    double *acc1 = acc0 + cap_owned, *acc2 = acc1 + cap_owned, *acc3 = acc2 + cap_owned;
    double *red = acc3 + cap_owned;
// ... 229 lines not shown
                }
                __syncthreads();
                peer_put_finish(*lag.put, lag, put_seq, put_off, lag.wait_end - lag.wait_begin, red);
                return;
            }
        }
    } else {
    typedef unsigned int u32x4 __attribute__((ext_vector_type(4)));
    typedef unsigned int u32x2 __attribute__((ext_vector_type(2)));
    constexpr bool kWide = sizeof(V2) == 16;
    __amdgpu_buffer_rsrc_t rx = __builtin_amdgcn_make_buffer_rsrc((void *)gx_free, 0, 0x7FFFFFF0, 0x00020000);
    __amdgpu_buffer_rsrc_t ru = __builtin_amdgcn_make_buffer_rsrc((void *)gu_free, 0, 0x7FFFFFF0, 0x00020000);
#pragma unroll
    for (int j = 0; j < NPT; ++j) {
        const int l = tid + j * BLOCK;
        if (l < n_owned) {
            if (gx_free && s[j].x >= 0) {
                V2 v;
                v.x = acc0[l]; v.y = acc1[l];
                if (kWide) __builtin_amdgcn_raw_buffer_store_b128(*reinterpret_cast<const u32x4 *>(&v), rx, s[j].x * 16, 0, SP);
                else __builtin_amdgcn_raw_buffer_store_b64(*reinterpret_cast<const u32x2 *>(&v), rx, s[j].x * 8, 0, SP);
            }
            if (gu_free && s[j].y >= 0) {
                V2 v;
                v.x = acc2[l]; v.y = acc3[l];
                if (kWide) __builtin_amdgcn_raw_buffer_store_b128(*reinterpret_cast<const u32x4 *>(&v), ru, s[j].y * 16, 0, SP);
                else __builtin_amdgcn_raw_buffer_store_b64(*reinterpret_cast<const u32x2 *>(&v), ru, s[j].y * 8, 0, SP);
            }
        }
    }
    }
    if (tid == 0) {
        double tile_e = 0.0;
#pragma unroll
        for (int w = 0; w < BLOCK / 64; ++w) tile_e += red[w];
        partials[slot] = tile_e;
    }
    if (pd.span && tid == 0) {
        __builtin_amdgcn_s_waitcnt(0x0F70);
        pd.span[2 * (size_t)(tile_begin + slot)] = t_start;
        pd.span[2 * (size_t)(tile_begin + slot) + 1] = __builtin_amdgcn_s_memrealtime();
    }
}

constexpr int kPairCapN = 656, kPairCapO = 560;
template <int BLK, int NPT, int EPT, int CAPO, bool HASB, bool PHYS, typename V2, bool ADAM, bool CHAIN, int SP = 16>
static void launch_pair_inst2(const TileLaunch &A, const LagSum &lag, const AdamFuse &af) {
    constexpr int CAPN = CAPO > 0 ? kPairCapN : 0;
    const size_t lds = CAPO > 0 ? (size_t)(CAPN * 32 + CAPO * 32 + 128) : A.lds;
    if constexpr (!HASB && !PHYS && !CHAIN) {
        if (lag.pg_blocks) {
            hipLaunchKernelGGL((tri3_energy_pair_kernel<BLK, NPT, EPT, 4, CAPO, HASB, PHYS, V2, ADAM, CHAIN, CAPN, SP, true>), dim3(A.grid), dim3(BLK), lds, A.s,
                               A.pd, A.tile_begin, (V2 *)const_cast<void *>(A.x_free), (const V2 *)A.x_fixed, (V2 *)const_cast<void *>(A.u_free),
                               (const V2 *)A.u_fixed, A.k, A.T_edge, A.tc, A.partials, (V2 *)A.gx, (V2 *)A.gu, A.max_nodes,
                               CAPO > 0 ? CAPO : A.max_owned, A.skip_edges, lag, af, A.col_stride);
            return;
        }
    }
    hipLaunchKernelGGL((tri3_energy_pair_kernel<BLK, NPT, EPT, 4, CAPO, HASB, PHYS, V2, ADAM, CHAIN, CAPN, SP>), dim3(A.grid), dim3(BLK), lds, A.s,
                       A.pd, A.tile_begin, (const V2 *)A.x_free, (const V2 *)A.x_fixed, (const V2 *)A.u_free,
                       (const V2 *)A.u_fixed, A.k, A.T_edge, A.tc, A.partials, (V2 *)A.gx, (V2 *)A.gu, A.max_nodes,
                       CAPO > 0 ? CAPO : A.max_owned, A.skip_edges, lag, af, A.col_stride);
}
template <int BLK, int NPT, int EPT, int CAPO, bool HASB, bool PHYS, typename V2, bool ADAM>
static void launch_pair_inst(const TileLaunch &A, const LagSum &lag, const AdamFuse &af) {
#ifdef HFEM_LAB
    if (A.chain) { launch_pair_inst2<BLK, NPT, EPT, CAPO, HASB, PHYS, V2, ADAM, true>(A, lag, af); return; }
#endif
    launch_pair_inst2<BLK, NPT, EPT, CAPO, HASB, PHYS, V2, ADAM, false>(A, lag, af);
}

int launch_tri3_pair(const hfem_plan *plan, TileLaunch A, int mode, bool hasb, bool phys, const LagSum &lag,
                     const AdamFuse &af) {
    const HostPlan &h = plan->host;
    if (!h.paired || !plan->d_elem_pack_hi) return 0;
    A.pd = plan_dev(plan);
    A.pd.span = A.span;
    A.max_nodes = h.max_nodes; A.max_owned = h.max_owned; A.lds = (size_t)plan->lds_bytes;
    A.col_stride = h.col_stride;
    if (A.chain < 0) A.chain = h.n_chained > 0 ? 1 : 0;
#ifndef HFEM_LAB
    if (A.chain) return 0;
#endif
    if (h.pair_block == 512) {
        if (h.max_nodes > 2 * 512 || h.max_rows > 2 || A.chain) return 0;
        if (mode == 0) {
            if (h.max_owned <= kPairCapO && h.max_nodes <= kPairCapN) launch_pair_inst2<512, 2, 2, 560, false, false, double2, false, false>(A, lag, af);
            else launch_pair_inst2<512, 2, 2, 0, false, false, double2, false, false>(A, lag, af);
            return 1;
        }
        if (mode == 1) {
            if (phys) launch_pair_inst2<512, 2, 2, 0, true, true, double2, false, false>(A, lag, af);
            else launch_pair_inst2<512, 2, 2, 0, true, false, double2, false, false>(A, lag, af);
            return 1;
        }
        if (mode == 2) { launch_pair_inst2<512, 2, 2, 0, false, false, float2, false, false>(A, lag, af); return 1; }
        if (mode == 3) {
            if (hasb) launch_pair_inst2<512, 2, 2, 0, true, false, double2, true, false>(A, lag, af);
            else launch_pair_inst2<512, 2, 2, 0, false, false, double2, true, false>(A, lag, af);
            return 1;
        }
        if (mode == 4) {
            if (hasb) launch_pair_inst2<512, 2, 2, 0, true, false, float2, true, false>(A, lag, af);
            else launch_pair_inst2<512, 2, 2, 0, false, false, float2, true, false>(A, lag, af);
            return 1;
        }
        return 0;
    }
    const bool cc = h.max_owned <= kPairCapO && h.max_nodes <= kPairCapN;
    const int npt = h.max_nodes <= 3 * 256 ? 3 : 4;
    const int ept = h.max_rows > 0 ? h.max_rows : 1;
    if (h.max_nodes > 4 * 256 || ept > 6) return 0;
#define HFEM_PAIR_EPT(NPT, CO, HB, PH, V, AD)                                                    \
    switch (ept) {                                                                               \
        case 1: case 2: case 3: launch_pair_inst<256, NPT, 3, CO, HB, PH, V, AD>(A, lag, af); return 1; \
        case 4: launch_pair_inst<256, NPT, 4, CO, HB, PH, V, AD>(A, lag, af); return 1;           \
        default: launch_pair_inst<256, NPT, 6, CO, HB, PH, V, AD>(A, lag, af); return 1;          \
    }
    const bool nt = plan->tune.store_policy == 2 && !A.chain && ept <= 4;
#define HFEM_PAIR_NT(NPT, CO, V)                                                                              \
    {                                                                                                         \
        if (ept <= 3) launch_pair_inst2<256, NPT, 3, CO, false, false, V, false, false, 2>(A, lag, af);      \
        else launch_pair_inst2<256, NPT, 4, CO, false, false, V, false, false, 2>(A, lag, af);               \
        return 1;                                                                                             \
    }
    if (mode == 0 && nt) {
        if (cc && npt == 3) HFEM_PAIR_NT(3, 560, double2)
        if (npt == 3) HFEM_PAIR_NT(3, 0, double2)
        HFEM_PAIR_NT(4, 0, double2)
    }
    if (mode == 2 && nt) {
        if (npt == 3) HFEM_PAIR_NT(3, 0, float2)
        HFEM_PAIR_NT(4, 0, float2)
    }
#undef HFEM_PAIR_NT
    if (mode == 0) {
#ifdef HFEM_LAB
        const int sp = plan->tune.store_policy;
        if (cc && npt == 3 && ept <= 3 && sp != 16 && !A.chain && !lag.pg_blocks) {
            const size_t lds = (size_t)(kPairCapN * 32 + kPairCapO * 32 + 128);
#define HFEM_PAIR_SP(SPV)                                                                                                  \
    hipLaunchKernelGGL((tri3_energy_pair_kernel<256, 3, 3, 4, 560, false, false, double2, false, false, kPairCapN, SPV>),  \
                       dim3(A.grid), dim3(256), lds, A.s, A.pd, A.tile_begin, (const double2 *)A.x_free,                   \
                       (const double2 *)A.x_fixed, (const double2 *)A.u_free, (const double2 *)A.u_fixed, A.k, A.T_edge,   \
                       A.tc, A.partials, (double2 *)A.gx, (double2 *)A.gu, A.max_nodes, 560, A.skip_edges, lag, af,         \
                       A.col_stride)
            switch (sp) {
                case 0: HFEM_PAIR_SP(0); return 1;
                case 17: HFEM_PAIR_SP(17); return 1;
                case 18: HFEM_PAIR_SP(18); return 1;
                default: break;
            }
#undef HFEM_PAIR_SP
        }
#endif
        if (cc && npt == 3) HFEM_PAIR_EPT(3, 560, false, false, double2, false)
        if (npt == 3) HFEM_PAIR_EPT(3, 0, false, false, double2, false)
        HFEM_PAIR_EPT(4, 0, false, false, double2, false)
    } else if (mode == 1) {
        if (phys) launch_pair_inst<256, 4, 6, 0, true, true, double2, false>(A, lag, af);
        else launch_pair_inst<256, 4, 6, 0, true, false, double2, false>(A, lag, af);
        return 1;
    } else if (mode == 2) {
        if (npt == 3) HFEM_PAIR_EPT(3, 0, false, false, float2, false)
        HFEM_PAIR_EPT(4, 0, false, false, float2, false)
    } else if (mode == 3) {
// ... 14 lines not shown
```

hidenn_fem_amd/csrc/tri3_pair_pipe.hip:

```cpp
#ifdef HFEM_LAB
#include <hip/hip_runtime.h>

#include "hfem_device.h"
#include "hfem_plan_dev.h"

namespace hfem {

typedef __attribute__((address_space(3))) void lds_void_pp_t;

__device__ __forceinline__ void pp_glds16(const void *gsrc, unsigned lds_dst) {
    unsigned keep;
    asm volatile("s_mov_b32 %0, m0\n\ts_mov_b32 m0, %2\n\ts_nop 0\n\tglobal_load_lds_dwordx4 %1, off\n\ts_mov_b32 m0, %0"
                 : "=&s"(keep)
                 : "v"(gsrc), "s"(lds_dst)
                 : "memory");
}
__device__ __forceinline__ unsigned pp_lds_addr(const void *p) { return (unsigned)(size_t)(lds_void_pp_t *)p; }

template <int BLOCK, int NPT, int EPT, int WPS>
__global__ __launch_bounds__(BLOCK, WPS) void tri3_energy_pair_pipe_kernel(
    PlanDev pd, int tile_begin, int n_tiles, int tpw, const double2 *__restrict__ x_free, const double2 *__restrict__ x_fixed,
    const double2 *__restrict__ u_free, const double2 *__restrict__ u_fixed, Tri3Consts k,
    const double4 *__restrict__ T_edge, double4 Tconst, double *__restrict__ partials,
    double2 *__restrict__ gx_free, double2 *__restrict__ gu_free, int cap_nodes, int cap_owned, int skip_edges,
    LagSum lag, int col_stride) {
    extern __shared__ double2 lds[];
    double *acc0 = reinterpret_cast<double *>(lds + 4 * cap_nodes);
    double *acc1 = acc0 + cap_owned, *acc2 = acc1 + cap_owned, *acc3 = acc2 + cap_owned;
    double *red = acc3 + cap_owned;
    int *dcache = reinterpret_cast<int *>(red + 8);

    const int tid = threadIdx.x, lane = tid & 63;
    const int n_wg = (int)gridDim.x - (lag.prev ? 1 : 0);
    if (lag.prev && (int)blockIdx.x == n_wg) {
        double v = 0.0;
        if (tid < 256)
            for (int i = tid; i < lag.prev_n; i += 256) v += lag.prev[i];
        const double tot = block_sum(v, red);
        if (tid == 0) lag.out[0] = tot;
        return;
    }
    const int wg = xcd_tile(blockIdx.x, n_wg);
    const int t_first = wg * tpw, t_end = min(t_first + tpw, n_tiles);
    if (t_first >= t_end) return;

    typedef unsigned int u32x4 __attribute__((ext_vector_type(4)));
    __amdgpu_buffer_rsrc_t rx = __builtin_amdgcn_make_buffer_rsrc((void *)gx_free, 0, 0x7FFFFFF0, 0x00020000);
    __amdgpu_buffer_rsrc_t ru = __builtin_amdgcn_make_buffer_rsrc((void *)gu_free, 0, 0x7FFFFFF0, 0x00020000);

    int2 s[NPT], sn[NPT];
    uint32_t w0[EPT], w1[EPT], wn0[EPT], wn1[EPT];
    int n_node, n_owned, n_elem, n_edge, edge_off;

#define HFEM_PP_INDEX(T, S, A, B)                                                                    \
    {                                                                                                 \
        const int2 *src_ = pd.node_src + (size_t)(tile_begin + (T)) * pd.node_stride;                 \
        const size_t rec_ = (size_t)(tile_begin + (T)) * pd.elem_stride;                              \
        _Pragma("unroll") for (int j = 0; j < NPT; ++j) S[j] = src_[min(tid + j * BLOCK, pd.node_stride - 1)]; \
        _Pragma("unroll") for (int j = 0; j < EPT; ++j) {                                             \
            const size_t i_ = rec_ + min(tid + j * col_stride, pd.elem_stride - 1);                   \
            A[j] = pd.elem_pack[i_];                                                                  \
            B[j] = pd.elem_pack_hi[i_];                                                               \
        }                                                                                             \
    }
#define HFEM_PP_GATHER(S, NN, BUF)                                                                    \
    _Pragma("unroll") for (int j = 0; j < NPT; ++j) {                                                \
        const int l_ = tid + j * BLOCK;                                                               \
        if (l_ < (NN)) {                                                                              \
            double2 *bx_ = lds + (BUF) * 2 * cap_nodes;                                               \
            const unsigned dx_ = __builtin_amdgcn_readfirstlane(pp_lds_addr(bx_ + (l_ - lane)));            \
            const unsigned du_ = __builtin_amdgcn_readfirstlane(pp_lds_addr(bx_ + cap_nodes + (l_ - lane))); \
            pp_glds16(S[j].x >= 0 ? x_free + S[j].x : x_fixed + ~S[j].x, dx_);                        \
            pp_glds16(S[j].y >= 0 ? u_free + S[j].y : u_fixed + ~S[j].y, du_);                        \
        }                                                                                             \
    }
    auto add_row = [&](int l, const double2 gx, const double2 gu) {
        unsafeAtomicAdd(&acc0[l], gx.x); unsafeAtomicAdd(&acc1[l], gx.y);
        unsafeAtomicAdd(&acc2[l], gu.x); unsafeAtomicAdd(&acc3[l], gu.y);
    };

    HFEM_PP_INDEX(t_first, s, w0, w1)
    if (tid < 8 * (t_end - t_first)) dcache[tid] = reinterpret_cast<const int *>(pd.tiles + tile_begin + t_first)[tid];
    {
        const TileDesc d = pd.tiles[tile_begin + t_first];
        n_node = d.n_node; n_owned = d.n_owned; n_elem = d.n_elem; n_edge = skip_edges ? 0 : d.n_edge; edge_off = d.edge_off;
    }
    HFEM_PP_GATHER(s, n_node, 0)
#pragma unroll
    for (int j = 0; j < NPT; ++j) {
        const int l = tid + j * BLOCK;
        if (l < n_owned) { acc0[l] = 0.0; acc1[l] = 0.0; acc2[l] = 0.0; acc3[l] = 0.0; }
    }
#pragma unroll
    for (int j = 0; j < EPT; ++j)
        if (!(tid < col_stride && tid + j * col_stride < n_elem)) { w0[j] = kSkipBit; w1[j] = 0u; }
    asm volatile("s_waitcnt vmcnt(0)" ::: "memory");
    __syncthreads();

    for (int t = t_first; t < t_end; ++t) {
        const int cur = (t - t_first) & 1;
// ... 136 lines not shown
```

hidenn_fem_amd/plan.py:

```python
from __future__ import annotations

import ctypes as C
import hashlib
import os
import tempfile
from typing import Optional

import numpy as np
import torch

from . import _lib

EXPORT_IDS = {"tile_desc": 0, "elem_pack": 1, "node_src": 2, "edge_pack": 3, "edge_gid": 4, "elem_gid": 5,
              "stamps": 6, "elem_pack_hi": 7, "tile_chunks": 8, "elem_gid_b": 9, "shard_desc": 10,
              "owned_node_ids": 11}


_PLAN_OPTIONS = (b"plan_elem_order", b"plan_node_cap", b"plan_shards", b"plan_pair_block", b"plan_chunk_cap", b"plan_curve",
                 b"plan_snap", b"plan_read_pack", b"tiled_block", b"store_policy", b"tiled_fast", b"fast_const_caps")


def _np(a, dtype):
    if a is None:
        return None
    if isinstance(a, torch.Tensor):
        a = a.detach().cpu().numpy()
    return np.ascontiguousarray(a, dtype=dtype)


def row_maps(free_mask: np.ndarray):
    free_mask = np.asarray(free_mask, dtype=bool)
    src = np.empty(free_mask.shape[0], dtype=np.int32)
    src[free_mask] = np.arange(int(free_mask.sum()), dtype=np.int32)
    src[~free_mask] = -1 - np.arange(int((~free_mask).sum()), dtype=np.int32)
    return src


def model_plan(model, tile_elems, paired: bool):
    plan = model.tile_plan(tile_elems)
    if bool(plan.stats["paired"]) == bool(paired):
        return plan
    key = (str(model.device), int(tile_elems), "paired" if paired else "single")
    if key not in model._plans:
        model._plans[key] = TilePlan(model.connectivity, model.Nnodes, coords_hint=model.initial_node_coords,
                                     x_src=model._x_src, u_src=model._u_src, edges=model.neumann_edges, tile_elems=tile_elems,
                                     device=model.device, elem_order=5 if paired else 3, nodes_per_elem=3)
    return model._plans[key]


class TilePlan:

    def __init__(self, connectivity, n_nodes: int, coords_hint=None, x_src=None, u_src=None,
                 edges=None, tile_elems: int = 0, device: Optional[torch.device] = None,
                 elem_order: Optional[int] = None, nodes_per_elem: int = 3, shards: int = 1,
                 pair_block: Optional[int] = None, cache_dir: Optional[str] = None):
        if nodes_per_elem not in (3, 4):
            raise ValueError("nodes_per_elem must be 3 (TRI3) or 4 (QUAD4)")
        self.nodes_per_elem = nodes_per_elem
        conn = _np(connectivity, np.int64).reshape(-1, nodes_per_elem)
        hint = _np(coords_hint, np.float64)
        xs, us = _np(x_src, np.int32), _np(u_src, np.int32)
        ed = _np(edges, np.int64)
        ed = None if ed is None else ed.reshape(-1, 2)
        if hint is not None and hint.shape != (n_nodes, 2):
            raise ValueError("coords_hint must be [n_nodes, 2]")
        for m in (xs, us):
            if m is not None and m.shape != (n_nodes,):
                raise ValueError("x_src / u_src must be [n_nodes]")
        self.device = device
        self.n_nodes, self.n_elems = int(n_nodes), int(conn.shape[0])
        self.n_edges = 0 if ed is None else int(ed.shape[0])
        self._h = C.c_void_p()
        dev = -1 if device is None else _lib.dev_index(device)

        def p(a):
            return None if a is None or a.size == 0 else a.ctypes.data_as(C.c_void_p)

        L = _lib.lib()
        wanted = {b"plan_elem_order": elem_order, b"plan_shards": int(shards) if int(shards) != 1 else None,
                  b"plan_pair_block": pair_block}
        cache_dir = cache_dir if cache_dir is not None else os.environ.get("HFEM_PLAN_CACHE") or None
        self.cache = None
        blob_path = None
        if cache_dir:
            hsh = hashlib.blake2b(digest_size=20)
            opts = {n: L.hfem_get_option(n) for n in _PLAN_OPTIONS}
            opts.update({k: int(v) for k, v in wanted.items() if v is not None})
            hsh.update(repr((L.hfem_version(), self.n_nodes, self.n_elems, nodes_per_elem, int(tile_elems),
                             sorted(opts.items()))).encode())
            for a_ in (conn, hint, xs, us, ed):
                hsh.update(b"-" if a_ is None else memoryview(a_).cast("B"))
            blob_path = os.path.join(cache_dir, f"plan_{hsh.hexdigest()}.bin")
            if os.path.exists(blob_path):
                try:
                    self._load_blob(np.fromfile(blob_path, dtype=np.uint8), dev)
                    self.cache = "hit"
                except RuntimeError:
                    self._h = C.c_void_p()
        if not self._h:
            prev = {}
            try:
                for name, val in wanted.items():
                    if val is not None:
                        prev[name] = L.hfem_get_option(name)
                        _lib.check(L.hfem_set_option(name, int(val)), "hfem_set_option")
                rc = L.hfem_plan_create_ex(dev, p(conn), self.n_elems, self.n_nodes, nodes_per_elem, p(hint), p(xs),
                                           p(us), p(ed), self.n_edges, int(tile_elems), C.byref(self._h))
            finally:
                for name, val in prev.items():
                    L.hfem_set_option(name, val)
            _lib.check(rc, "hfem_plan_create")
            if blob_path is not None:
                self.cache = "miss"
                os.makedirs(cache_dir, exist_ok=True)
                fd, tmp = tempfile.mkstemp(dir=cache_dir, suffix=".tmp")
                try:
                    with os.fdopen(fd, "wb") as f:
                        self.to_bytes().tofile(f)
                    os.replace(tmp, blob_path)
                except OSError:
                    try:
                        os.unlink(tmp)
                    except OSError:
                        pass
        self._finish_init()

    def _finish_init(self):
        st = _lib.PlanStats()
        _lib.check(_lib.lib().hfem_plan_get_stats(self._h, C.byref(st)), "hfem_plan_get_stats")
        self.stats = st.as_dict()
        self.n_tiles = self.stats["n_tiles"]
        self.n_nodes, self.n_elems, self.n_edges = self.stats["n_nodes"], self.stats["n_elems"], self.stats["n_edges"]
        self.nodes_per_elem = self.stats["nodes_per_elem"]

    @property
    def handle(self):
        return self._h

    def to_bytes(self) -> np.ndarray:
        L = _lib.lib()
        n = L.hfem_plan_serialize(self._h, None, 0)
        if n < 0:
            _lib.check(-1, "hfem_plan_serialize")
        out = np.empty(int(n), dtype=np.uint8)
        if L.hfem_plan_serialize(self._h, out.ctypes.data_as(C.c_void_p), n) != n:
            _lib.check(-1, "hfem_plan_serialize")
        return out

    def _load_blob(self, blob: np.ndarray, dev: int):
        blob = np.ascontiguousarray(blob, dtype=np.uint8)
        self._h = C.c_void_p()
        _lib.check(_lib.lib().hfem_plan_deserialize(dev, blob.ctypes.data_as(C.c_void_p), blob.size, C.byref(self._h)),
                   "hfem_plan_deserialize")

    @classmethod
    def from_bytes(cls, blob, device: Optional[torch.device] = None) -> "TilePlan":
        self = cls.__new__(cls)
        self.device, self.cache = device, None
        self._load_blob(np.frombuffer(blob, dtype=np.uint8) if not isinstance(blob, np.ndarray) else blob,
                        -1 if device is None else _lib.dev_index(device))
        self._finish_init()
        return self

# ... 79 lines not shown
```

include/hidenn_fem.h:

```cpp
#ifndef HIDENN_FEM_H
#define HIDENN_FEM_H

#include <stdint.h>

#ifdef __cplusplus
extern "C" {
#endif

#define HFEM_VERSION 114

int hfem_version(void);
const char *hfem_last_error(void);
int hfem_device_count(void);


int hfem_tri3_energy_atomic(int device, const double *X, const double *U,
                            const int32_t *conn, int64_t e_begin, int64_t e_end, int64_t nn,
                            const double mat[4], double W, const double Bk[6],
                            double *loss_acc, double *gX, double *gU, void *stream);

int hfem_edge2_energy_atomic(int device, const double *X, const double *U,
                             const int32_t *edges, int64_t ned, const double *T,
                             const double Tconst[4], double *loss_acc, double *gX,
                             double *gU, void *stream);

typedef struct hfem_plan hfem_plan;

typedef struct hfem_plan_stats {
    int64_t n_elems, n_nodes, n_edges;
    int32_t n_tiles, tile_elems;
    int64_t tile_elem_total;
    int64_t tile_node_total;
    int32_t max_tile_nodes, max_tile_owned, max_tile_elems, max_tile_edges;
    int64_t device_bytes;
    int32_t lds_bytes;
    int32_t shards;
    int32_t threads_per_tile;
    int32_t paired;
    int32_t slot_rows;
    int32_t store_policy;
    int32_t nodes_per_elem;
    double row_line_factor;
} hfem_plan_stats;

int hfem_plan_create(int device, const int64_t *conn, int64_t ne, int64_t nn,
                     const double *coords_hint, const int32_t *x_src, const int32_t *u_src,
                     const int64_t *edges, int64_t ned, int32_t tile_elems,
                     hfem_plan **out);
int hfem_plan_create_ex(int device, const int64_t *conn, int64_t ne, int64_t nn, int32_t nodes_per_elem,
                        const double *coords_hint, const int32_t *x_src, const int32_t *u_src,
                        const int64_t *edges, int64_t ned, int32_t tile_elems, hfem_plan **out);
int hfem_plan_destroy(hfem_plan *plan);
int hfem_plan_get_stats(const hfem_plan *plan, hfem_plan_stats *out);
int64_t hfem_plan_export(const hfem_plan *plan, int which, void *buf, int64_t cap_elems);

int64_t hfem_plan_serialize(const hfem_plan *plan, void *buf, int64_t cap_bytes);
int hfem_plan_deserialize(int device, const void *blob, int64_t n_bytes, hfem_plan **out);

#define HFEM_FLAG_NO_GX 1
#define HFEM_FLAG_NO_GU 2
#define HFEM_FLAG_NO_EDGES 4
#define HFEM_FLAG_NO_LOSS_SUM 8
#define HFEM_FLAG_PHYSICAL_GRAD 64
#define HFEM_FLAG_DETERMINISTIC 128
#define HFEM_FLAG_SUM_PREVIOUS 32

#define HFEM_FLAG_PEER_GET 512
#define HFEM_FLAG_PEER_PUT 2048
#define HFEM_FLAG_FP32_MATH 1024
#define HFEM_FLAG_SAME_BANK 256

int hfem_tri3_energy_plan(hfem_plan *plan, const double *x_free, const double *x_fixed,
                          const double *u_free, const double *u_fixed,
                          const double mat[4], double W, const double Bk[6],
                          const double *T_edge, const double Tconst[4],
                          int32_t tile_begin, int32_t tile_end, double *loss_out,
                          double *gx_free, double *gu_free, int32_t flags, void *stream);
int hfem_tri3_energy_plan_f32(hfem_plan *plan, const float *x_free, const float *x_fixed,
                              const float *u_free, const float *u_fixed,
                              const double mat[4], double W, const double Bk[6],
                              const double *T_edge, const double Tconst[4],
                              int32_t tile_begin, int32_t tile_end, double *loss_out,
                              float *gx_free, float *gu_free, int32_t flags, void *stream);
int hfem_tri3_energy_adam_step(hfem_plan *plan, const double *x_free, const double *x_fixed,
                               const double *u_free, const double *u_fixed, const double mat[4], double W,
                               const double *T_edge, const double Tconst[4], double *x_out, double *u_out,
                               double *m_x, double *v_x, double *m_u, double *v_u, double lr_x, double lr_u,
                               double beta1, double beta2, double eps, const double *bc_dev,
                               double *loss_out, int32_t flags, void *stream);
int hfem_tri3_energy_adam_step_ex(hfem_plan *plan, int32_t dtype, const void *x_free, const void *x_fixed,
                                  const void *u_free, const void *u_fixed, const double mat[4], double W,
                                  const double Bk[6], const double *T_edge, const double Tconst[4], void *x_out,
                                  void *u_out, void *m_x, void *v_x, void *m_u, void *v_u, double lr_x, double lr_u,
                                  double beta1, double beta2, double eps, const double *bc_dev, int32_t tile_begin,
                                  int32_t tile_end, double *loss_out, int32_t flags, void *stream);
int hfem_adam_prep(int device, int64_t *step_dev, double beta1, double beta2, double *bc_dev, void *stream);
int hfem_plan_loss_sum(hfem_plan *plan, int32_t tile_begin, int32_t tile_end, double *loss_out, void *stream);

int hfem_plan_set_span_stamps(hfem_plan *plan, uint64_t *dev_buf, int64_t n_slots);

int hfem_set_option(const char *name, int value);
int hfem_get_option(const char *name);

int hfem_tri3_eval_fwd(int device, const double *X, const double *U, const int32_t *conn,
                       const double *x_eval, const int64_t *elem_id, int64_t m,
                       double *u_h, double *detJ, double *grad_u, void *stream);
int hfem_tri3_eval_bwd(int device, const double *X, const double *U, const int32_t *conn,
                       const double *x_eval, const int64_t *elem_id, int64_t m,
                       const double *cu, const double *cd, const double *cg,
                       double *gX, double *gU, void *stream);
#define HFEM_GRAD_REFERENCE 0
#define HFEM_GRAD_PHYSICAL 1
int hfem_tri3_eval_fwd_conv(int device, const double *X, const double *U, const int32_t *conn,
                            const double *x_eval, const int64_t *elem_id, int64_t m,
                            double *u_h, double *detJ, double *grad_u, int32_t convention, void *stream);
int hfem_tri3_eval_bwd_conv(int device, const double *X, const double *U, const int32_t *conn,
                            const double *x_eval, const int64_t *elem_id, int64_t m,
                            const double *cu, const double *cd, const double *cg,
                            double *gX, double *gU, int32_t convention, void *stream);
int hfem_edge2_eval_fwd(int device, const double *X, const double *U, const int32_t *edges,
                        const double *xi, const int64_t *edge_id, int64_t m,
                        double *u_h, double *ds, void *stream);
int hfem_edge2_eval_bwd(int device, const double *X, const double *U, const int32_t *edges,
                        const double *xi, const int64_t *edge_id, int64_t m,
                        const double *cu, const double *cds, double *gX, double *gU,
// ... 347 lines not shown
```

Measured before the change: 119.3 billion element-evals/s.

## Add two-stage paired TRI3 kernel storing deep-node gradients early

Adds a plan option that renumbers each tile's owned nodes into deep, shallow and late classes. Slots touching only early nodes are packed into the first wave of work, so gradients of nodes that are already complete can be written to global memory while later slots are still being computed. A new staged kernel overlaps these early stores with the remaining computation and async global-to-LDS loads. The cost is a greedy O(n^2) planning pass and extra plan complexity. The new path runs only when the two_stage option is enabled.

```diff
diff --git a/hidenn_fem_amd/_lib.py b/hidenn_fem_amd/_lib.py
--- a/hidenn_fem_amd/_lib.py
+++ b/hidenn_fem_amd/_lib.py
@@ -22,6 +22,7 @@
         ("device_bytes", _i64), ("lds_bytes", _i32),
         ("shards", _i32), ("threads_per_tile", _i32), ("paired", _i32), ("slot_rows", _i32),
         ("store_policy", _i32), ("nodes_per_elem", _i32), ("row_line_factor", _f64),
+        ("two_stage", _i32), ("reserved1", _i32), ("deep_rows", _i64),
     ]
 
     def as_dict(self):
diff --git a/hidenn_fem_amd/csrc/build.py b/hidenn_fem_amd/csrc/build.py
--- a/hidenn_fem_amd/csrc/build.py
+++ b/hidenn_fem_amd/csrc/build.py
@@ -7,8 +7,8 @@
 
 HERE = os.path.dirname(os.path.abspath(__file__))
 ROOT = os.path.dirname(os.path.dirname(HERE))
-SOURCES = ["plan.cpp", "mg.cpp", "tri3_energy.hip", "tri3_stream.hip", "tri3_pair.hip", "tri3_pair_f32.hip", "tri3_pair_lab.hip", "tri3_pair_pipe.hip", "tri3_det.hip", "tri3_eval.hip", "line_rect.hip", "quad4.hip", "optim.hip", "exchange.hip", "peer.hip", "post.hip", "recover.hip", "lbfgs.hip", "cg.hip", "tri3_cg.hip", "quad4_cg.hip", "mesh_guard.hip", "amg.cpp", "tri3_amg.hip", "tri3_hyper.hip", "tri3_hyper_cg.hip", "quad4_hyper.hip", "quad4_hyper_cg.hip", "modal.hip"]
-HEADERS = ["hfem_common.h", "hfem_amg.h", "hfem_amg_hyper_dev.h", "hfem_cg_dev.h", "hfem_crossing_dev.h", "hfem_device.h", "hfem_hyper_dev.h", "hfem_mesh_dev.h", "hfem_mesh_elem_dev.h", "hfem_plan_dev.h", "hfem_quad4_dev.h", "hfem_quad4_hyper_dev.h", "hfem_recover_hyper_dev.h", "tri3_energy_lab.inc", os.path.join(ROOT, "include", "hidenn_fem.h")]
+SOURCES = ["plan.cpp", "mg.cpp", "tri3_energy.hip", "tri3_stream.hip", "tri3_pair.hip", "tri3_pair_staged.hip", "tri3_pair_f32.hip", "tri3_pair_lab.hip", "tri3_pair_pipe.hip", "tri3_det.hip", "tri3_eval.hip", "line_rect.hip", "quad4.hip", "optim.hip", "exchange.hip", "peer.hip", "post.hip", "recover.hip", "lbfgs.hip", "cg.hip", "tri3_cg.hip", "quad4_cg.hip", "mesh_guard.hip", "amg.cpp", "tri3_amg.hip", "tri3_hyper.hip", "tri3_hyper_cg.hip", "quad4_hyper.hip", "quad4_hyper_cg.hip", "modal.hip"]
+HEADERS = ["hfem_common.h", "hfem_amg.h", "hfem_amg_hyper_dev.h", "hfem_cg_dev.h", "hfem_crossing_dev.h", "hfem_device.h", "hfem_hyper_dev.h", "hfem_mesh_dev.h", "hfem_mesh_elem_dev.h", "hfem_pair_dev.h", "hfem_plan_dev.h", "hfem_quad4_dev.h", "hfem_quad4_hyper_dev.h", "hfem_recover_hyper_dev.h", "tri3_energy_lab.inc", os.path.join(ROOT, "include", "hidenn_fem.h")]
 OUT = os.path.join(HERE, "libhidenn_hip.so")
 OUT_LAB = os.path.join(HERE, "libhidenn_hip_lab.so")
 ARCH = "gfx950"
diff --git a/hidenn_fem_amd/csrc/hfem_common.h b/hidenn_fem_amd/csrc/hfem_common.h
--- a/hidenn_fem_amd/csrc/hfem_common.h
+++ b/hidenn_fem_amd/csrc/hfem_common.h
@@ -68,13 +68,16 @@
     int32_t pair_block = 256;
     std::vector<int32_t> owned_gid;
     std::vector<int32_t> owned_gid_by_slot;
+    bool two_stage = false;
+    int64_t n_deep_total = 0;
 };
+constexpr int32_t kStageEarlyIds = 512;
 constexpr int kChunks = 3;
 
 int build_host_plan(const int64_t *conn, int npe, int64_t ne, int64_t nn, const double *coords,
                     const int32_t *x_src, const int32_t *u_src, const int64_t *edges,
                     int64_t ned, int32_t tile_elems, int32_t node_cap, int elem_order, int32_t chunk_cap,
-                    HostPlan &out, int32_t pair_block = 256, int32_t shards = 1);
+                    HostPlan &out, int32_t pair_block = 256, int32_t shards = 1, bool two_stage = false);
 
 void serialize_host_plan(const HostPlan &h, const void *trailer, size_t trailer_bytes, std::vector<unsigned char> &blob);
 int deserialize_host_plan(const void *blob, size_t n, HostPlan &h, void *trailer, size_t trailer_bytes);
diff --git a/hidenn_fem_amd/csrc/hfem_pair_dev.h b/hidenn_fem_amd/csrc/hfem_pair_dev.h
--- /dev/null
+++ b/hidenn_fem_amd/csrc/hfem_pair_dev.h
@@ -0,0 +1,100 @@
+#pragma once
+#include <hip/hip_runtime.h>
+
+#include <type_traits>
+
+#include "hfem_device.h"
+#include "hfem_plan_dev.h"
+
+namespace hfem {
+
+struct PairAcc {
+    double *a0, *a1, *a2, *a3;
+};
+__device__ __forceinline__ void pair_add_row(const PairAcc &A, int l, const double2 gx, const double2 gu) {
+    unsafeAtomicAdd(&A.a0[l], gx.x); unsafeAtomicAdd(&A.a1[l], gx.y);
+    unsafeAtomicAdd(&A.a2[l], gu.x); unsafeAtomicAdd(&A.a3[l], gu.y);
+}
+
+template <bool HASB, bool PHYS>
+__device__ __forceinline__ void pair_slot(const uint32_t p, const uint32_t q, const double2 *nd_xy, const double2 *nd_uv,
+                                          const PairAcc &A, const int n_owned, const Tri3Consts &k, double &e_loc) {
+    if (!(p & kSkipBit)) {
+        const int ln = (int)(p & kLocalMask), lb = (int)((p >> kLocalBits) & kLocalMask),
+                  lc = (int)((p >> (2 * kLocalBits)) & kLocalMask);
+        const double2 Xn = nd_xy[ln], Un = nd_uv[ln], Xc = nd_xy[lc], Uc = nd_uv[lc];
+        double2 sxn, sun, sxc, suc;
+        {
+            double2 gx[3], gu[3];
+            const double e = tri3_element<true, HASB, PHYS>(Xn, nd_xy[lb], Xc, Un, nd_uv[lb], Uc, k, gx, gu);
+            if (p & kHomeBit) e_loc += e;
+            if (lb < n_owned) pair_add_row(A, lb, gx[1], gu[1]);
+            sxn = gx[0]; sun = gu[0]; sxc = gx[2]; suc = gu[2];
+        }
+        if (q & kHasBBit) {
+            const int ld = (int)(q & kLocalMask);
+            double2 gx[3], gu[3];
+            const double e = tri3_element<true, HASB, PHYS>(Xn, Xc, nd_xy[ld], Un, Uc, nd_uv[ld], k, gx, gu);
+            if (q & kHomeBBit) e_loc += e;
+            if (ld < n_owned) pair_add_row(A, ld, gx[2], gu[2]);
+            sxn.x += gx[0].x; sxn.y += gx[0].y; sun.x += gu[0].x; sun.y += gu[0].y;
+            sxc.x += gx[1].x; sxc.y += gx[1].y; suc.x += gu[1].x; suc.y += gu[1].y;
+        }
+        if (ln < n_owned) pair_add_row(A, ln, sxn, sun);
+        if (lc < n_owned) pair_add_row(A, lc, sxc, suc);
+    }
+}
+
+template <int BLOCK>
+__device__ __forceinline__ void pair_edges(const PlanDev &pd, const int edge_off, const int n_edge, const int tid,
+                                           const uint32_t edge_rec, const int edge_id, const double4 *__restrict__ T_edge,
+                                           const double4 Tconst, const double2 *nd_xy, const double2 *nd_uv, const PairAcc &A,
+                                           const int n_owned, double &e_loc) {
+    for (int i = tid; i < n_edge; i += BLOCK) {
+        const uint32_t p = i == tid ? edge_rec : pd.edge_pack[edge_off + i];
+        const int l0 = (int)(p & kLocalMask), l1 = (int)((p >> kLocalBits) & kLocalMask);
+        double4 tt = Tconst;
+        if (T_edge) tt = T_edge[i == tid ? edge_id : pd.edge_gid[edge_off + i]];
+        double2 gx[2], gu[2];
+        const double wk = edge2_element<true>(nd_xy[l0], nd_xy[l1], nd_uv[l0], nd_uv[l1], tt, gx, gu);
+        if (p & kHomeBit) e_loc -= wk;
+        if (l0 < n_owned) pair_add_row(A, l0, gx[0], gu[0]);
+        if (l1 < n_owned) pair_add_row(A, l1, gx[1], gu[1]);
+    }
+}
+
+template <typename V2, int SP>
+__device__ __forceinline__ void pair_store_row(const __amdgpu_buffer_rsrc_t rx, const __amdgpu_buffer_rsrc_t ru,
+                                               const bool have_gx, const bool have_gu, const int sx, const int su,
+                                               const int l, const PairAcc &A) {
+    typedef unsigned int u32x4 __attribute__((ext_vector_type(4)));
+    typedef unsigned int u32x2 __attribute__((ext_vector_type(2)));
+    constexpr bool kWide = sizeof(V2) == 16;
+    if (have_gx && sx >= 0) {
+        V2 v;
+        v.x = A.a0[l]; v.y = A.a1[l];
+        if (kWide) __builtin_amdgcn_raw_buffer_store_b128(*reinterpret_cast<const u32x4 *>(&v), rx, sx * 16, 0, SP);
+        else __builtin_amdgcn_raw_buffer_store_b64(*reinterpret_cast<const u32x2 *>(&v), rx, sx * 8, 0, SP);
+    }
+    if (have_gu && su >= 0) {
+        V2 v;
+        v.x = A.a2[l]; v.y = A.a3[l];
+        if (kWide) __builtin_amdgcn_raw_buffer_store_b128(*reinterpret_cast<const u32x4 *>(&v), ru, su * 16, 0, SP);
+        else __builtin_amdgcn_raw_buffer_store_b64(*reinterpret_cast<const u32x2 *>(&v), ru, su * 8, 0, SP);
+    }
+}
+__device__ __forceinline__ __amdgpu_buffer_rsrc_t pair_grad_rsrc(void *p) {
+    return __builtin_amdgcn_make_buffer_rsrc(p, 0, 0x7FFFFFF0, 0x00020000);
+}
+
+typedef __attribute__((address_space(3))) void lds_void_pp_t;
+__device__ __forceinline__ void pp_glds16(const void *gsrc, unsigned lds_dst) {
+    unsigned keep;
+    asm volatile("s_mov_b32 %0, m0\n\ts_mov_b32 m0, %2\n\ts_nop 0\n\tglobal_load_lds_dwordx4 %1, off\n\ts_mov_b32 m0, %0"
+                 : "=&s"(keep)
+                 : "v"(gsrc), "s"(lds_dst)
+                 : "memory");
+}
+__device__ __forceinline__ unsigned pp_lds_addr(const void *p) { return (unsigned)(size_t)(lds_void_pp_t *)p; }
+
+}
diff --git a/hidenn_fem_amd/csrc/hfem_plan_dev.h b/hidenn_fem_amd/csrc/hfem_plan_dev.h
--- a/hidenn_fem_amd/csrc/hfem_plan_dev.h
+++ b/hidenn_fem_amd/csrc/hfem_plan_dev.h
@@ -307,6 +307,7 @@
 };
 int launch_tri3_pair(const hfem_plan *plan, TileLaunch A, int mode, bool hasb, bool phys, const LagSum &lag,
                      const AdamFuse &af);
+int launch_tri3_pair_staged(const hfem_plan *plan, TileLaunch A, const LagSum &lag);
 int launch_tri3_pair_f32(const hfem_plan *plan, TileLaunch A, bool hasb, const LagSum &lag, const AdamFuse *adam = nullptr);
 #ifdef HFEM_LAB
 int launch_tri3_pair_lab(const hfem_plan *plan, TileLaunch A, int mode, bool hasb, bool phys, const LagSum &lag,
diff --git a/hidenn_fem_amd/csrc/plan.cpp b/hidenn_fem_amd/csrc/plan.cpp
--- a/hidenn_fem_amd/csrc/plan.cpp
+++ b/hidenn_fem_amd/csrc/plan.cpp
@@ -450,7 +450,7 @@
 int try_build(const int64_t *conn, int npe, int64_t ne, int64_t nn, const double *xy, const int32_t *x_src,
               const int32_t *u_src, const int64_t *edges, int64_t ned, int32_t T, int32_t node_cap,
               const std::vector<int32_t> &order, int elem_order, int32_t chunk_cap, int32_t pair_block, int32_t shards,
-              HostPlan &P) {
+              bool two_stage, HostPlan &P) {
     std::vector<int64_t> bounds;
     cut_tiles(conn, npe, ne, nn, order, T, node_cap, bounds);
     const int32_t nt_main = ne > 0 ? (int32_t)bounds.size() - 1 : 0;
@@ -671,6 +671,62 @@
                     }
                 }
             std::stable_sort(slots.begin(), slots.end(), [](const std::array<int32_t, 2> &x, const std::array<int32_t, 2> &y) { return (x[1] >= 0) > (y[1] >= 0); });
+            std::vector<char> early_slot;
+            int32_t n_deep = 0;
+            if (two_stage && elem_order == 5 && pair_block == 256 && nloc > kStageEarlyIds) {
+                const int S = (int)slots.size(), n_own = d.n_owned;
+                const int need = std::min(S, (int)pair_block);
+                std::vector<std::array<int32_t, 4>> sl(S);
+                for (int si = 0; si < S; ++si) {
+                    const int64_t ea = telems[slots[si][0]];
+                    sl[si] = {lid[conn[3 * ea]], lid[conn[3 * ea + 1]], lid[conn[3 * ea + 2]],
+                              slots[si][1] >= 0 ? lid[conn[3 * (int64_t)telems[slots[si][1]] + 2]] : -1};
+                }
+                std::vector<char> late_o(n_own, 0), slot_late(S, 0);
+                for (int si = 0; si < S; ++si)
+                    for (int q = 0; q < 4; ++q) slot_late[si] |= sl[si][q] >= n_own && sl[si][q] >= kStageEarlyIds;
+                std::vector<int32_t> cost(n_own), lateadj(n_own);
+                for (int pick = 0; pick < n_own - kStageEarlyIds; ++pick) {
+                    std::fill(cost.begin(), cost.end(), 0);
+                    std::fill(lateadj.begin(), lateadj.end(), 0);
+                    for (int si = 0; si < S; ++si)
+                        for (int q = 0; q < 4; ++q) {
+                            const int32_t l = sl[si][q];
+                            if (l >= 0 && l < n_own) ++(slot_late[si] ? lateadj : cost)[l];
+                        }
+                    int best = -1;
+                    for (int l = 0; l < n_own; ++l) {
+                        if (late_o[l]) continue;
+                        if (best < 0 || cost[l] < cost[best] || (cost[l] == cost[best] && lateadj[l] >= lateadj[best])) best = l;
+                    }
+                    late_o[best] = 1;
+                    for (int si = 0; si < S; ++si)
+                        for (int q = 0; q < 4; ++q) slot_late[si] |= sl[si][q] == best;
+                }
+                early_slot.assign(S, 0);
+                int got = 0;
+                for (int si = 0; si < S && got < need; ++si)
+                    if (!slot_late[si]) { early_slot[si] = 1; ++got; }
+                if (got < need) return 2;
+                std::vector<char> shallow(n_own, 0);
+                for (int si = 0; si < S; ++si)
+                    if (!early_slot[si])
+                        for (int q = 0; q < 4; ++q)
+                            if (sl[si][q] >= 0 && sl[si][q] < n_own) shallow[sl[si][q]] = 1;
+                for (int64_t i = edg_ptr[t]; i < edg_ptr[t + 1]; ++i)
+                    for (int q = 0; q < 2; ++q) {
+                        const int32_t l = lid[edges[2 * (int64_t)tedge[i] + q]];
+                        if (l < n_own) shallow[l] = 1;
+                    }
+                std::vector<int32_t> renum;
+                renum.reserve(n_own);
+                for (int cls = 0; cls < 3; ++cls)
+                    for (int l = 0; l < n_own; ++l)
+                        if ((late_o[l] ? 2 : (shallow[l] ? 1 : 0)) == cls) renum.push_back(own_order[l]);
+                for (int l = 0; l < n_own; ++l) n_deep += !late_o[l] && !shallow[l];
+                own_order.swap(renum);
+                for (int l = 0; l < n_own; ++l) lid[own_order[l]] = l;
+            }
             std::vector<std::array<int32_t, 4>> items(slots.size());
             for (size_t s_ = 0; s_ < slots.size(); ++s_) {
                 const int64_t ea = telems[slots[s_][0]];
@@ -769,7 +825,21 @@
                 while (!order_s.empty() && order_s.back() < 0) order_s.pop_back();
                 P.max_rows = std::max(P.max_rows, rows_used);
             } else {
-            if (g_halfwave_pack) {
+            if (!early_slot.empty()) {
+                std::vector<std::array<int32_t, 4>> part;
+                std::vector<int32_t> idx, o;
+                for (int pass = 0; pass < 2; ++pass) {
+                    part.clear(); idx.clear(); o.clear();
+                    for (size_t si = 0; si < slots.size(); ++si)
+                        if ((early_slot[si] != 0) == (pass == 0)) { part.push_back(items[si]); idx.push_back((int32_t)si); }
+                    if (part.empty()) continue;
+                    pack_slot_halfwaves(part, d.n_owned, o);
+                    if (pass == 1 && (int32_t)order_s.size() != pair_block) return 2;
+                    for (int32_t v : o) order_s.push_back(v < 0 ? -1 : idx[v]);
+                }
+                d.pad = pair_block | (n_deep << 16);
+                P.n_deep_total += n_deep;
+            } else if (g_halfwave_pack) {
                 pack_slot_halfwaves(items, d.n_owned, order_s);
             } else {
                 std::vector<std::array<int32_t, 4>> part(items.begin(), items.begin() + n_pair);
@@ -841,6 +911,7 @@
     }
     P.shards = shards;
     P.pair_block = pair_block;
+    P.two_stage = two_stage && P.paired && elem_order == 5 && pair_block == 256;
     P.shard_desc.clear();
     {
         std::vector<TileDesc> sorted_tiles;
@@ -898,11 +969,12 @@
     {
         int32_t cs = 0;
         if (P.paired) {
-            for (int32_t t = 0; t < nt; ++t) cs = std::max(cs, P.tiles[t].pad);
+            for (int32_t t = 0; t < nt; ++t) cs = std::max(cs, P.tiles[t].pad & 0xFFFF);
             P.max_elems = 0;
             for (int32_t t = 0; t < nt; ++t) {
                 const TileDesc &d = P.tiles[t];
-                const int32_t ne_new = d.n_elem > 0 ? ((d.n_elem - 1) / d.pad) * cs + (d.n_elem - 1) % d.pad + 1 : 0;
+                const int32_t pad = d.pad & 0xFFFF;
+                const int32_t ne_new = d.n_elem > 0 ? ((d.n_elem - 1) / pad) * cs + (d.n_elem - 1) % pad + 1 : 0;
                 P.max_elems = std::max(P.max_elems, ne_new);
             }
             P.col_stride = cs;
@@ -917,9 +989,10 @@
         for (int32_t t = 0; t < nt; ++t) {
             TileDesc &d = P.tiles[t];
             const size_t so = (size_t)d.elem_off, dn = (size_t)t * stride, n = (size_t)d.n_elem;
+            const size_t pad = cs > 0 ? (size_t)(d.pad & 0xFFFF) : 1;
             int32_t n_new = 0;
             for (size_t i = 0; i < n; ++i) {
-                const size_t k = cs > 0 ? (i / d.pad) * cs + i % d.pad : i;
+                const size_t k = cs > 0 ? (i / pad) * cs + i % pad : i;
                 ep[dn + k] = P.elem_pack[so + i];
                 eg[dn + k] = P.elem_gid[so + i];
                 if (hi) eh[dn + k] = P.elem_pack_hi[so + i];
@@ -929,7 +1002,7 @@
             real += d.n_elem;
             d.elem_off = (int32_t)dn;
             d.n_elem = n_new;
-            if (cs > 0) d.pad = cs;
+            if (cs > 0) d.pad = cs | (d.pad & ~0xFFFF);
         }
         P.elem_pack.swap(ep); P.elem_gid.swap(eg); P.elem_pack_hi.swap(eh); P.elem_gid_b.swap(egb);
         P.elem_stride = (int32_t)stride;
@@ -952,7 +1025,7 @@
 int build_host_plan(const int64_t *conn, int npe, int64_t ne, int64_t nn, const double *coords,
                     const int32_t *x_src, const int32_t *u_src, const int64_t *edges,
                     int64_t ned, int32_t tile_elems, int32_t node_cap, int elem_order, int32_t chunk_cap,
-                    HostPlan &out, int32_t pair_block, int32_t shards) {
+                    HostPlan &out, int32_t pair_block, int32_t shards, bool two_stage) {
     if (pair_block != 256 && pair_block != 512) { set_error("plan: pair_block must be 256 or 512"); return -1; }
     if (shards < 1 || shards > 4096) { set_error("plan: shards must be in [1, 4096]"); return -1; }
     if (npe != 3 && npe != 4) { set_error("plan: nodes per element must be 3 (TRI3) or 4 (QUAD4)"); return -1; }
@@ -972,8 +1045,11 @@
     std::vector<int32_t> order;
     morton_order(conn, npe, ne, nn, coords, order);
     for (int32_t T = tile_elems; T >= 16; T = (T * 2) / 3) {
-        const int rc = try_build(conn, npe, ne, nn, coords, x_src, u_src, edges, ned, T, node_cap, order, elem_order, chunk_cap,
-                                 pair_block, shards, out);
+        int rc = try_build(conn, npe, ne, nn, coords, x_src, u_src, edges, ned, T, node_cap, order, elem_order, chunk_cap,
+                           pair_block, shards, two_stage, out);
+        if (rc == 2)
+            rc = try_build(conn, npe, ne, nn, coords, x_src, u_src, edges, ned, T, node_cap, order, elem_order, chunk_cap,
+                           pair_block, shards, false, out);
         if (rc == 0 && npe == 4 && out.max_elems > kMaxQuadSlots) continue;
         if (rc == 0 && out.paired && out.max_rows > (pair_block == 512 ? 2 : kMaxRows)) continue;
         if (rc == 0) {
@@ -993,11 +1069,12 @@
 }
 
 namespace {
-constexpr uint32_t kBlobVersion = 1;
+constexpr uint32_t kBlobVersion = 2;
 struct BlobScalars {
     int64_t ne, nn, ned, elem_records, node_records, n_pairs, n_chained;
     int32_t tile_elems, npe, node_stride, elem_stride, col_stride, max_nodes, max_owned, max_elems, max_edges, max_rows,
-        max_chunk_elems, shards, pair_block, paired;
+        max_chunk_elems, shards, pair_block, paired, two_stage, reserved;
+    int64_t n_deep_total;
 };
 uint64_t fnv1a(const unsigned char *p, size_t n) {
     uint64_t h = 1469598103934665603ull;
@@ -1043,6 +1120,7 @@
     sc.node_stride = h.node_stride; sc.elem_stride = h.elem_stride; sc.col_stride = h.col_stride; sc.max_nodes = h.max_nodes;
     sc.max_owned = h.max_owned; sc.max_elems = h.max_elems; sc.max_edges = h.max_edges; sc.max_rows = h.max_rows;
     sc.max_chunk_elems = h.max_chunk_elems; sc.shards = h.shards; sc.pair_block = h.pair_block; sc.paired = h.paired ? 1 : 0;
+    sc.two_stage = h.two_stage ? 1 : 0; sc.n_deep_total = h.n_deep_total;
     b.insert(b.end(), (const unsigned char *)&sc, (const unsigned char *)&sc + sizeof(sc));
     b.resize((b.size() + 7) & ~(size_t)7, 0);
     std::vector<int32_t> td((const int32_t *)h.tiles.data(), (const int32_t *)h.tiles.data() + 8 * h.tiles.size());
@@ -1078,6 +1156,7 @@
     h.node_stride = sc.node_stride; h.elem_stride = sc.elem_stride; h.col_stride = sc.col_stride; h.max_nodes = sc.max_nodes;
     h.max_owned = sc.max_owned; h.max_elems = sc.max_elems; h.max_edges = sc.max_edges; h.max_rows = sc.max_rows;
     h.max_chunk_elems = sc.max_chunk_elems; h.shards = sc.shards; h.pair_block = sc.pair_block; h.paired = sc.paired != 0;
+    h.two_stage = sc.two_stage != 0; h.n_deep_total = sc.n_deep_total;
     std::vector<int32_t> td;
     bool ok = get_vec(p, n - 8, at, td) && td.size() % 8 == 0;
     ok = ok && get_vec(p, n - 8, at, h.elem_pack) && get_vec(p, n - 8, at, h.elem_pack_hi) && get_vec(p, n - 8, at, h.elem_gid) &&
@@ -1103,7 +1182,8 @@
         if (d.n_node < 0 || d.n_node > h.max_nodes || d.n_owned < 0 || d.n_owned > d.n_node || d.n_elem < 0 || d.n_elem > h.max_elems ||
             d.node_off < 0 || (size_t)d.node_off + d.n_node > h.node_src.size() / 2 || d.elem_off < 0 ||
             (size_t)d.elem_off + d.n_elem > h.elem_pack.size() || d.n_edge < 0 || d.edge_off < 0 ||
-            (size_t)d.edge_off + d.n_edge > h.edge_pack.size()) {
+            (size_t)d.edge_off + d.n_edge > h.edge_pack.size() ||
+            (h.paired && ((d.pad >> 16) < 0 || (d.pad >> 16) > std::min(d.n_owned, kStageEarlyIds) || (!h.two_stage && (d.pad >> 16))))) {
             set_error("plan blob: tile descriptor out of range");
             return -1;
         }
diff --git a/hidenn_fem_amd/csrc/tri3_energy.hip b/hidenn_fem_amd/csrc/tri3_energy.hip
--- a/hidenn_fem_amd/csrc/tri3_energy.hip
+++ b/hidenn_fem_amd/csrc/tri3_energy.hip
@@ -404,6 +404,7 @@
     std::atomic<int> plan_chunk_cap{512};
     std::atomic<int> plan_shards{1};
     std::atomic<int> plan_pair_block{-1};
+    std::atomic<int> plan_two_stage{-1};
 } g_def;
 
 #ifdef HFEM_LAB
@@ -411,6 +412,8 @@
 #include "tri3_energy_lab.inc"
 #undef HFEM_LAB_SECTION
 #endif
+
+constexpr bool kTwoStageAuto = false;
 
 hfem_plan::Tune current_tune() {
     hfem_plan::Tune t;
@@ -715,9 +718,17 @@
 #endif
     const bool auto_order = order < 0;
     if (auto_order) order = nodes_per_elem == 3 ? 5 : 3;
+    const int two_stage_opt = g_def.plan_two_stage.load();
+    const bool stage_auto = two_stage_opt < 0 && kTwoStageAuto && nodes_per_elem == 3 && order == 5 && pair_block == 256 && per_shard > 600000;
     if (build_host_plan(conn, nodes_per_elem, ne, nn, coords_hint, x_src, u_src, edges, ned, tile_elems, node_cap, order,
-                        g_def.plan_chunk_cap.load(), p->host, pair_block, shards))
+                        g_def.plan_chunk_cap.load(), p->host, pair_block, shards, two_stage_opt == 1 || stage_auto))
         return -1;
+    if (stage_auto && p->host.two_stage && p->host.max_rows != 3) {
+        p->host = HostPlan();
+        if (build_host_plan(conn, nodes_per_elem, ne, nn, coords_hint, x_src, u_src, edges, ned, tile_elems, node_cap, order,
+                            g_def.plan_chunk_cap.load(), p->host, pair_block, shards, false))
+            return -1;
+    }
     if (auto_order && p->host.paired && 2 * p->host.n_pairs * 10 < 7 * ne) {
         p->host = HostPlan();
         if (build_host_plan(conn, nodes_per_elem, ne, nn, coords_hint, x_src, u_src, edges, ned, tile_elems, node_cap, 3,
@@ -807,6 +818,8 @@
     out->store_policy = plan->tune.store_policy;
     out->nodes_per_elem = h.npe;
     out->row_line_factor = plan->row_line_factor;
+    out->two_stage = h.two_stage ? 1 : 0;
+    out->deep_rows = h.n_deep_total;
     return 0;
 }
 
@@ -1211,6 +1224,9 @@
     } else if (n == "plan_pair_block") {
         HFEM_ARG_CHECK(value == -1 || value == 256 || value == 512, "plan_pair_block: -1 (auto), 256 or 512 threads per tile");
         g_def.plan_pair_block = value;
+    } else if (n == "plan_two_stage") {
+        HFEM_ARG_CHECK(value >= -1 && value <= 1, "plan_two_stage: -1 (auto), 0 (off) or 1 (wherever the plan can be staged)");
+        g_def.plan_two_stage = value;
     } else if (n == "plan_curve") {
         HFEM_ARG_CHECK(value == 0 || value == 1, "plan_curve: 0 Morton, 1 Hilbert");
         set_plan_curve(value);
@@ -1248,6 +1264,7 @@
     if (n == "plan_chunk_cap") return g_def.plan_chunk_cap.load();
     if (n == "plan_shards") return g_def.plan_shards.load();
     if (n == "plan_pair_block") return g_def.plan_pair_block.load();
+    if (n == "plan_two_stage") return g_def.plan_two_stage.load();
     if (n == "plan_snap") return g_def.plan_snap.load();
     if (n == "plan_read_pack") return g_def.plan_read_pack.load();
     if (n == "lab_build") {
diff --git a/hidenn_fem_amd/csrc/tri3_pair.hip b/hidenn_fem_amd/csrc/tri3_pair.hip
--- a/hidenn_fem_amd/csrc/tri3_pair.hip
+++ b/hidenn_fem_amd/csrc/tri3_pair.hip
@@ -335,6 +335,7 @@
 #ifndef HFEM_LAB
     if (A.chain) return 0;
 #endif
+    if (mode == 0 && h.two_stage && !A.chain && launch_tri3_pair_staged(plan, A, lag)) return 1;
     if (h.pair_block == 512) {
         if (h.max_nodes > 2 * 512 || h.max_rows > 2 || A.chain) return 0;
         if (mode == 0) {
diff --git a/hidenn_fem_amd/csrc/tri3_pair_pipe.hip b/hidenn_fem_amd/csrc/tri3_pair_pipe.hip
--- a/hidenn_fem_amd/csrc/tri3_pair_pipe.hip
+++ b/hidenn_fem_amd/csrc/tri3_pair_pipe.hip
@@ -1,21 +1,9 @@
 #ifdef HFEM_LAB
 #include <hip/hip_runtime.h>
 
-#include "hfem_device.h"
-#include "hfem_plan_dev.h"
+#include "hfem_pair_dev.h"
 
 namespace hfem {
-
-typedef __attribute__((address_space(3))) void lds_void_pp_t;
-
-__device__ __forceinline__ void pp_glds16(const void *gsrc, unsigned lds_dst) {
-    unsigned keep;
-    asm volatile("s_mov_b32 %0, m0\n\ts_mov_b32 m0, %2\n\ts_nop 0\n\tglobal_load_lds_dwordx4 %1, off\n\ts_mov_b32 m0, %0"
-                 : "=&s"(keep)
-                 : "v"(gsrc), "s"(lds_dst)
-                 : "memory");
-}
-__device__ __forceinline__ unsigned pp_lds_addr(const void *p) { return (unsigned)(size_t)(lds_void_pp_t *)p; }
 
 template <int BLOCK, int NPT, int EPT, int WPS>
 __global__ __launch_bounds__(BLOCK, WPS) void tri3_energy_pair_pipe_kernel(
diff --git a/hidenn_fem_amd/csrc/tri3_pair_staged.hip b/hidenn_fem_amd/csrc/tri3_pair_staged.hip
--- /dev/null
+++ b/hidenn_fem_amd/csrc/tri3_pair_staged.hip
@@ -0,0 +1,174 @@
+#include <hip/hip_runtime.h>
+
+#include "hfem_pair_dev.h"
+
+namespace hfem {
+
+constexpr int kStagedCapN = 656, kStagedCapO = 560, kStagedEarly = 512;
+template <int CAPO, int SP>
+__global__ __launch_bounds__(256, 4) void tri3_energy_pair_staged_kernel(
+    PlanDev pd, int tile_begin, const double2 *__restrict__ x_free, const double2 *__restrict__ x_fixed,
+    const double2 *__restrict__ u_free, const double2 *__restrict__ u_fixed, Tri3Consts k,
+    const double4 *__restrict__ T_edge, double4 Tconst, double *__restrict__ partials,
+    double2 *__restrict__ gx_free, double2 *__restrict__ gu_free, int cap_nodes, int cap_owned_rt, int skip_edges,
+    LagSum lag, int col_stride) {
+    constexpr int BLOCK = 256, NPT = 3, EPT = 3;
+    constexpr int NREG = 2;
+    static_assert(kStagedEarly == 2 * BLOCK, "the late node row is row 2");
+    const int cap_owned = CAPO > 0 ? CAPO : cap_owned_rt;
+    const int cap_n = CAPO > 0 ? kStagedCapN : cap_nodes;
+    extern __shared__ double2 lds[];
+    double2 *nd_xy = lds;
+    double2 *nd_uv = lds + cap_n;
+    double *acc0 = reinterpret_cast<double *>(lds + 2 * cap_n);
+    const PairAcc acc{acc0, acc0 + cap_owned, acc0 + 2 * cap_owned, acc0 + 3 * cap_owned};
+    double *red = acc0 + 4 * cap_owned;
+
+    const int tid = threadIdx.x;
+    const int bid = (int)blockIdx.x;
+    const int n_launch = (int)gridDim.x - (lag.prev ? 1 : 0);
+    const bool sum_wg = lag.prev && bid == n_launch;
+    const int slot = xcd_tile(sum_wg ? n_launch - 1 : bid, n_launch);
+    mem_phase_begin();
+    const unsigned long long t_start = __builtin_amdgcn_s_memrealtime();
+    int2 s[NPT];
+    const int2 *src = pd.node_src + (size_t)(tile_begin + slot) * pd.node_stride;
+#pragma unroll
+    for (int j = 0; j < NPT; ++j) s[j] = src[min(tid + j * BLOCK, pd.node_stride - 1)];
+    const TileDesc d = pd.tiles[tile_begin + slot];
+    uint32_t w0[EPT], w1[EPT];
+    const size_t rec0 = (size_t)(tile_begin + slot) * pd.elem_stride;
+#pragma unroll
+    for (int j = 0; j < EPT; ++j) {
+        const size_t i = rec0 + min(tid + j * col_stride, pd.elem_stride - 1);
+        w0[j] = pd.elem_pack[i];
+        w1[j] = pd.elem_pack_hi[i];
+    }
+#pragma unroll
+    for (int j = 0; j < NPT; ++j) {
+        const int l = tid + j * BLOCK;
+        if ((CAPO > 0 && (j + 1) * BLOCK <= CAPO) || l < cap_owned) { acc.a0[l] = 0.0; acc.a1[l] = 0.0; acc.a2[l] = 0.0; acc.a3[l] = 0.0; }
+    }
+    __builtin_amdgcn_sched_barrier(0);
+    if (sum_wg) {
+        mem_phase_end();
+        double v = 0.0;
+        for (int i = tid; i < lag.prev_n; i += 256) v += lag.prev[i];
+        const double tot = block_sum(v, red);
+        if (tid == 0) lag.out[0] = tot;
+        return;
+    }
+    double2 vx[NREG], vu[NREG];
+#pragma unroll
+    for (int j = 0; j < NREG; ++j) {
+        vx[j] = *(s[j].x >= 0 ? x_free + s[j].x : x_fixed + ~s[j].x);
+        vu[j] = *(s[j].y >= 0 ? u_free + s[j].y : u_fixed + ~s[j].y);
+    }
+    __builtin_amdgcn_sched_barrier(0);
+    const int n_owned = d.n_owned;
+    const int n_deep = (int)((unsigned)d.pad >> 16);
+    const int n_edge = skip_edges ? 0 : d.n_edge;
+    uint32_t edge_rec = 0u;
+    int edge_id = 0;
+    if (tid < n_edge) {
+        edge_rec = pd.edge_pack[d.edge_off + tid];
+        if (T_edge) edge_id = pd.edge_gid[d.edge_off + tid];
+    }
+#pragma unroll
+    for (int j = 0; j < EPT; ++j)
+        if (!(tid < col_stride && tid + j * col_stride < d.n_elem)) { w0[j] = kSkipBit; w1[j] = 0u; }
+    asm volatile("s_waitcnt vmcnt(0)"
+                 :
+                 : "v"(s[0].x), "v"(s[0].y), "v"(s[1].x), "v"(s[1].y), "v"(s[2].x), "v"(s[2].y), "v"(w0[0]), "v"(w0[1]), "v"(w0[2]),
+                   "v"(w1[0]), "v"(w1[1]), "v"(w1[2]), "v"(vx[0].x), "v"(vx[0].y), "v"(vx[1].x), "v"(vx[1].y), "v"(vu[0].x),
+                   "v"(vu[0].y), "v"(vu[1].x), "v"(vu[1].y), "v"(edge_rec), "v"(edge_id)
+                 : "memory");
+#pragma unroll
+    for (int j = 0; j < NREG; ++j) {
+        const int l = tid + j * BLOCK;
+        if (l < d.n_node) {
+            nd_xy[l] = make_double2(vx[j].x, vx[j].y);
+            nd_uv[l] = make_double2(vu[j].x, vu[j].y);
+        }
+    }
+    __syncthreads();
+    {
+        const int l = tid + 2 * BLOCK;
+        if (l < d.n_node) {
+            const unsigned dx = __builtin_amdgcn_readfirstlane(pp_lds_addr(nd_xy + (l - (tid & 63))));
+            const unsigned du = __builtin_amdgcn_readfirstlane(pp_lds_addr(nd_uv + (l - (tid & 63))));
+            pp_glds16(s[2].x >= 0 ? x_free + s[2].x : x_fixed + ~s[2].x, dx);
+            pp_glds16(s[2].y >= 0 ? u_free + s[2].y : u_fixed + ~s[2].y, du);
+        }
+    }
+    mem_phase_end();
+
+    double e_loc = 0.0;
+    pair_slot<false, false>(w0[0], w1[0], nd_xy, nd_uv, acc, n_owned, k, e_loc);
+    asm volatile("s_waitcnt vmcnt(0)" ::: "memory");
+    __syncthreads();
+
+    const __amdgpu_buffer_rsrc_t rx = pair_grad_rsrc((void *)gx_free), ru = pair_grad_rsrc((void *)gu_free);
+    if (n_deep > 0) {
+        mem_phase_begin();
+#pragma unroll
+        for (int j = 0; j < 2; ++j) {
+            const int l = tid + j * BLOCK;
+            if (l < n_deep) pair_store_row<double2, SP>(rx, ru, gx_free != nullptr, gu_free != nullptr, s[j].x, s[j].y, l, acc);
+        }
+        mem_phase_end();
+    }
+#pragma unroll
+    for (int j = 1; j < EPT; ++j) pair_slot<false, false>(w0[j], w1[j], nd_xy, nd_uv, acc, n_owned, k, e_loc);
+    pair_edges<BLOCK>(pd, d.edge_off, n_edge, tid, edge_rec, edge_id, T_edge, Tconst, nd_xy, nd_uv, acc, n_owned, e_loc);
+    {
+        const double w = wave_sum_valu(e_loc);
+        if ((tid & 63) == 0) red[tid >> 6] = w;
+    }
+    mem_phase_begin();
+    __builtin_amdgcn_s_waitcnt(0x0F70);
+    __syncthreads();
+#pragma unroll
+    for (int j = 0; j < NPT; ++j) {
+        const int l = tid + j * BLOCK;
+        if (l >= n_deep && l < n_owned) pair_store_row<double2, SP>(rx, ru, gx_free != nullptr, gu_free != nullptr, s[j].x, s[j].y, l, acc);
+    }
+    if (tid == 0) {
+        double tile_e = 0.0;
+#pragma unroll
+        for (int w = 0; w < BLOCK / 64; ++w) tile_e += red[w];
+        partials[slot] = tile_e;
+    }
+    if (pd.span && tid == 0) {
+        __builtin_amdgcn_s_waitcnt(0x0F70);
+        pd.span[2 * (size_t)(tile_begin + slot)] = t_start;
+        pd.span[2 * (size_t)(tile_begin + slot) + 1] = __builtin_amdgcn_s_memrealtime();
+    }
+}
+
+template <int CAPO, int SP>
+static void launch_staged_inst(const TileLaunch &A, const LagSum &lag) {
+    const size_t lds = CAPO > 0 ? (size_t)(kStagedCapN * 32 + CAPO * 32 + 128) : A.lds;
+    hipLaunchKernelGGL((tri3_energy_pair_staged_kernel<CAPO, SP>), dim3(A.grid), dim3(256), lds, A.s, A.pd, A.tile_begin,
+                       (const double2 *)A.x_free, (const double2 *)A.x_fixed, (const double2 *)A.u_free,
+                       (const double2 *)A.u_fixed, A.k, A.T_edge, A.tc, A.partials, (double2 *)A.gx, (double2 *)A.gu,
+                       A.max_nodes, CAPO > 0 ? CAPO : A.max_owned, A.skip_edges, lag, A.col_stride);
+}
+
+int launch_tri3_pair_staged(const hfem_plan *plan, TileLaunch A, const LagSum &lag) {
+    const HostPlan &h = plan->host;
+    if (!h.paired || !h.two_stage || !plan->d_elem_pack_hi || h.pair_block != 256 || h.n_chained > 0 || lag.pg_blocks) return 0;
+    if (h.max_nodes > 3 * 256 || h.max_rows > 3 || h.col_stride != 256) return 0;
+    if (plan->tune.store_policy != 16 && plan->tune.store_policy != 2) return 0;
+    A.pd = plan_dev(plan);
+    A.pd.span = A.span;
+    A.max_nodes = h.max_nodes; A.max_owned = h.max_owned; A.lds = (size_t)plan->lds_bytes;
+    A.col_stride = h.col_stride;
+    const bool cc = h.max_owned <= kStagedCapO && h.max_nodes <= kStagedCapN;
+    const bool nt = plan->tune.store_policy == 2;
+    if (cc) { if (nt) launch_staged_inst<kStagedCapO, 2>(A, lag); else launch_staged_inst<kStagedCapO, 16>(A, lag); }
+    else { if (nt) launch_staged_inst<0, 2>(A, lag); else launch_staged_inst<0, 16>(A, lag); }
+    return 1;
+}
+
+}
diff --git a/hidenn_fem_amd/plan.py b/hidenn_fem_amd/plan.py
--- a/hidenn_fem_amd/plan.py
+++ b/hidenn_fem_amd/plan.py
@@ -17,7 +17,7 @@
 
 
 _PLAN_OPTIONS = (b"plan_elem_order", b"plan_node_cap", b"plan_shards", b"plan_pair_block", b"plan_chunk_cap", b"plan_curve",
-                 b"plan_snap", b"plan_read_pack", b"tiled_block", b"store_policy", b"tiled_fast", b"fast_const_caps")
+                 b"plan_snap", b"plan_read_pack", b"plan_two_stage", b"tiled_block", b"store_policy", b"tiled_fast", b"fast_const_caps")
 
 
 def _np(a, dtype):
@@ -53,7 +53,7 @@
     def __init__(self, connectivity, n_nodes: int, coords_hint=None, x_src=None, u_src=None,
                  edges=None, tile_elems: int = 0, device: Optional[torch.device] = None,
                  elem_order: Optional[int] = None, nodes_per_elem: int = 3, shards: int = 1,
-                 pair_block: Optional[int] = None, cache_dir: Optional[str] = None):
+                 pair_block: Optional[int] = None, cache_dir: Optional[str] = None, two_stage: Optional[int] = None):
         if nodes_per_elem not in (3, 4):
             raise ValueError("nodes_per_elem must be 3 (TRI3) or 4 (QUAD4)")
         self.nodes_per_elem = nodes_per_elem
@@ -78,7 +78,7 @@
 
         L = _lib.lib()
         wanted = {b"plan_elem_order": elem_order, b"plan_shards": int(shards) if int(shards) != 1 else None,
-                  b"plan_pair_block": pair_block}
+                  b"plan_pair_block": pair_block, b"plan_two_stage": two_stage}
         cache_dir = cache_dir if cache_dir is not None else os.environ.get("HFEM_PLAN_CACHE") or None
         self.cache = None
         blob_path = None
diff --git a/include/hidenn_fem.h b/include/hidenn_fem.h
--- a/include/hidenn_fem.h
+++ b/include/hidenn_fem.h
@@ -41,6 +41,9 @@
     int32_t store_policy;
     int32_t nodes_per_elem;
     double row_line_factor;
+    int32_t two_stage;
+    int32_t reserved1;
+    int64_t deep_rows;
 } hfem_plan_stats;
 
 int hfem_plan_create(int device, const int64_t *conn, int64_t ne, int64_t nn,
```

Result: faster. 120.9 billion element-evals/s (median of 5 runs) (+1.4%).
